# sThalham/PyraPose

Hardware: AMD Instinct MI355X
Metric: images/sec 640x480 fwd+bwd (train step: fwd + losses + bwd + clipnorm-Adam) (higher is better)
Workload: dtype bf16x3+f16c8

## Files before the change

include/pyrapose_hip.h:

```cpp
#ifndef PYRAPOSE_HIP_H
#define PYRAPOSE_HIP_H

#include <stddef.h>
#include <stdint.h>

#ifdef __cplusplus
extern "C" {
#endif

#define PP_OK 0
#define PP_ERR_ARG (-1)
#define PP_ERR_SHAPE (-2)
#define PP_ERR_ALIGN (-3)
#define PP_ERR_NOCTX (-4)
#define PP_ERR_UNSUPPORTED (-5)
#define PP_ERR_COMM (-6)

#define PP_MAX_SEG 5

typedef struct pp_ctx pp_ctx;

int pp_ctx_create(pp_ctx** out, int device, void* hip_stream);
void pp_ctx_destroy(pp_ctx* ctx);
int pp_ctx_set_stream(pp_ctx* ctx, void* hip_stream);
int pp_ctx_set_workspace(pp_ctx* ctx, void* device_buffer, size_t bytes);
int pp_ctx_set_split_capture(pp_ctx* ctx, void* hi, void* lo);
int pp_row_block_list(pp_ctx* ctx, const float* x, int rows, int ld, int cols, unsigned char* flags, int* list);
int pp_row_block_list_planes(pp_ctx* ctx, const void* x_hi, const void* x_lo, int rows, int ld, int cols, unsigned char* flags, int* list);
int pp_row_block_list_planes_within(pp_ctx* ctx, const void* x_hi, const void* x_lo, int rows, int ld, int cols, const unsigned char* within,
                                    unsigned char* flags, int* list);
int pp_ctx_set_epilogue_planes(pp_ctx* ctx, const void* add_hi, const void* add_lo, const void* mask_hi);
int pp_ctx_set_row_block_skip(pp_ctx* ctx, const unsigned char* flags, const int* list);
int pp_ctx_set_row_block_lazy(pp_ctx* ctx, int lazy_out, int lazy_in);
const char* pp_last_error_string(pp_ctx* ctx);
const char* pp_version(void);
int pp_device_info(pp_ctx* ctx, int* n_cu, char* name_host, int name_len);

typedef struct {
  int n_img;
  int n_seg;
  int h[PP_MAX_SEG];
  int w[PP_MAX_SEG];
} pp_rowspace;

typedef struct {
  pp_rowspace in;
  pp_rowspace out;
  int cin, cout;
  int kh, kw, stride;
  int pad_t, pad_l;
  int ld_x, ld_y, ld_w;
} pp_conv_desc;

int pp_conv2d_nhwc_fwd(pp_ctx* ctx, const pp_conv_desc* d, const float* x, const float* w,
                       const float* bias, const float* residual, int ld_res, int relu, float* y);

int pp_conv2d_nhwc_bwd_data(pp_ctx* ctx, const pp_conv_desc* d, const float* dy, const float* w,
                            const float* addend, int ld_add, const float* relu_src, int ld_rs, float* dx);

int pp_conv2d_nhwc_bwd_weight(pp_ctx* ctx, const pp_conv_desc* d, const float* x, const float* dy,
                              float* dw, float* dbias);

int pp_conv_split_weights_bf16x3(pp_ctx* ctx, const pp_conv_desc* d, const float* w, void* fwd_hi, void* fwd_lo,
                                 void* dgrad_hi, void* dgrad_lo);
typedef struct pp_split_job {
  const float* w;
  void* fwd_hi; void* fwd_lo; void* dg_hi; void* dg_lo;
  int taps, cin, cout, ld_w;
  int tile_begin, reserved;
} pp_split_job;
int pp_conv_split_weights_bf16x3_batch(pp_ctx* ctx, int n_jobs, const pp_split_job* jobs_dev, int total_tiles);
int pp_positive_row_blocks(pp_ctx* ctx, const pp_rowspace* rs, int A, int stride, const float* y_true, unsigned char* flags);
int pp_row_block_dilate(pp_ctx* ctx, const pp_conv_desc* d, const unsigned char* in_flags, unsigned char* out_flags);
int pp_ctx_set_row_block_out(pp_ctx* ctx, const unsigned char* flags, int* list);
int pp_split_planes_bf16x3(pp_ctx* ctx, size_t n, const float* src, void* hi, void* lo);
int pp_ctx_set_planes_format(pp_ctx* ctx, int fmt);
int pp_convert_planes(pp_ctx* ctx, size_t n, const void* src_hi, const void* src_lo, int src_fmt, void* dst_hi, void* dst_lo, int dst_fmt,
                      const float* scale2_dev, int scale_index, const void* relu_src_hi);
int pp_grad_scale_from_counts(pp_ctx* ctx, const int* counts_dev, int n_counts, float* scale2_dev);
int pp_grad_scale_from_counts_adj(pp_ctx* ctx, const int* counts_dev, int n_counts, float* scale2_dev, int log2_adjust);
int pp_split_planes_scaled_bf16x3(pp_ctx* ctx, size_t n, const float* src, void* hi, void* lo, const float* scale_dev);
int pp_ctx_set_grad_scale(pp_ctx* ctx, const float* scale2_dev);

int pp_conv2d_nhwc_fwd_bf16x3(pp_ctx* ctx, const pp_conv_desc* d, const float* x, const void* x_hi, const void* x_lo,
                              const void* w_fwd_hi, const void* w_fwd_lo, const float* bias, const float* residual,
                              int ld_res, int relu, float* y, void* y_hi, void* y_lo);
int pp_conv2d_nhwc_bwd_data_bf16x3(pp_ctx* ctx, const pp_conv_desc* d, const float* dy, const void* dy_hi,
                                   const void* dy_lo, const void* w_dgrad_hi, const void* w_dgrad_lo,
                                   const float* addend, int ld_add, const float* relu_src, int ld_rs, float* dx,
                                   void* dx_hi, void* dx_lo);
int pp_conv2d_nhwc_bwd_weight_bf16x3(pp_ctx* ctx, const pp_conv_desc* d, const float* x, const float* dy,
                                     const void* x_hi, const void* x_lo, const void* dy_hi, const void* dy_lo,
                                     float* dw, float* dbias);

typedef struct pp_comm pp_comm;
int pp_comm_available(void);
int pp_comm_unique_id(pp_ctx* ctx, void* id128);
int pp_comm_init(pp_ctx* ctx, int world, int rank, const void* id128, pp_comm** out);
int pp_comm_destroy(pp_comm* comm);
int pp_allreduce_bucket(pp_ctx* ctx, pp_comm* comm, float* buf, size_t count);
int pp_allreduce_counts(pp_ctx* ctx, pp_comm* comm, int* counts, int n);

int pp_maxpool3x3s2_fwd(pp_ctx* ctx, int n_img, int h, int w, int c, const float* x, int oh, int ow, float* y);
int pp_upsample_nearest_add_fwd(pp_ctx* ctx, int n_img, int sh, int sw, int th, int tw, int c,
                                const float* src, const float* other, float* out);
int pp_upsample_nearest_add_bwd(pp_ctx* ctx, int n_img, int sh, int sw, int th, int tw, int c,
                                const float* dtarget, const float* base, float* dsrc);
int pp_add_n(pp_ctx* ctx, size_t n, const float* a, const float* b, const float* c, float* out);
int pp_relu_fwd(pp_ctx* ctx, size_t n, const float* x, float* y);
typedef struct pp_tview {
  const float* f32;
  const void* hi;
  const void* lo;
} pp_tview;
int pp_add_n_v(pp_ctx* ctx, size_t n, const pp_tview* a, const pp_tview* b, const pp_tview* c, const pp_tview* out);
int pp_relu_fwd_v(pp_ctx* ctx, size_t n, const pp_tview* x, const pp_tview* y);
int pp_upsample_nearest_add_fwd_v(pp_ctx* ctx, int n_img, int sh, int sw, int th, int tw, int c, const pp_tview* src,
                                  const pp_tview* other, const pp_tview* out);
int pp_upsample_nearest_add_bwd_v(pp_ctx* ctx, int n_img, int sh, int sw, int th, int tw, int c, const pp_tview* dtarget,
                                  const pp_tview* base, const pp_tview* dsrc);
int pp_merge_planes_bf16x3(pp_ctx* ctx, size_t n, const void* hi, const void* lo, float* dst);
int pp_planes_stats(pp_ctx* ctx, const void* hi, const void* lo, long long rows, int ld, int cols, const unsigned char* within,
                    unsigned long long* stats5_dev);
int pp_pack_rgb_to_4(pp_ctx* ctx, size_t n_pixels, const float* x3, float* x4);
int pp_preprocess_caffe_u8(pp_ctx* ctx, int n_img, int H, int W, const int* sizes_hw_host, const unsigned char* images_u8,
                           float* x4);
int pp_warp_affine_u8(pp_ctx* ctx, int n_img, int H, int W, int channels, const double* mats_host, int interpolation, int border,
                      int cval, const unsigned char* src, unsigned char* dst);
int pp_resize_scale(int rows, int cols, int min_side, int max_side, double* scale);
int pp_resize_linear_u8(pp_ctx* ctx, int n_img, int SH, int SW, int channels, double scale, int DH, int DW, const unsigned char* src,
                        unsigned char* dst);
int pp_pack_rgb_to_4_padded(pp_ctx* ctx, int n_img, int H, int W, int Hp, int Wp, int pad, const float* x3, float* x4p);
int pp_preprocess_caffe_u8_padded(pp_ctx* ctx, int n_img, int H, int W, int Hp, int Wp, int pad, const int* sizes_hw_host,
                                  const unsigned char* images_u8, float* x4p);
int pp_stem7x7s2_fwd_bf16x3(pp_ctx* ctx, int n_img, int H, int W, int Hp, int Wp, const float* x4p, const void* w_hi,
                            const void* w_lo, int cout, const float* bias, int relu, float* y, int ld_y);

int pp_export_head(pp_ctx* ctx, const pp_rowspace* rs, int n_anchor, int n_val, const float* src, int ld,
                   int apply_sigmoid, float* out);

int pp_count_positives(pp_ctx* ctx, size_t rows_box, const float* y_box, size_t rows_cls, int c_cls,
                       const float* y_cls, size_t rows_mask, int c_mask, const float* y_mask, int* counts);
int pp_sigmoid_focal_fwd_bwd(pp_ctx* ctx, const pp_rowspace* rs, int n_anchor, int n_class,
                             const float* logits, int ld, const float* y_true, float alpha, float gamma,
                             const int* count, float loss_weight, float* loss_sum, float* dlogits);
int pp_orth_smoothl1_fwd_bwd(pp_ctx* ctx, const pp_rowspace* rs, int n_anchor, const float* pred, int ld,
                             const float* y_true, float weight, float sigma, const int* count,
                             float loss_weight, float* loss_sum, float* dpred);

typedef struct {
  long long offset;
  long long count;
  int ld;
  int trainable;
  long long scale_off;
  float l2;
} pp_param_desc;

typedef struct pp_optimizer pp_optimizer;
int pp_optimizer_create(pp_ctx* ctx, pp_optimizer** out, const pp_param_desc* descs_host, int n_desc,
                        long long total);
void pp_optimizer_destroy(pp_optimizer* opt);
int pp_grad_global_norm(pp_ctx* ctx, pp_optimizer* opt, const float* w_master, const float* g_eff,
                        const float* scales, float* gnorm_sq, float* l2_loss);
int pp_adam_step_clipnorm(pp_ctx* ctx, pp_optimizer* opt, float* w_master, float* w_eff, const float* g_eff,
                          const float* scales, float* m, float* v, const float* gnorm_sq, float lr,
                          float beta1, float beta2, float eps, float clipnorm, long long step);

int pp_generate_base_anchors_host(int base_size, const float* ratios_host, int n_ratios,
                                  const float* scales_host, int n_scales, double* out_host);
int pp_anchors_shift_f64(pp_ctx* ctx, int n_levels, const int* feat_h_host, const int* feat_w_host,
                         const int* strides_host, int n_anchor, const double* base_anchors_host,
                         double* anchors_out);
int pp_anchors_shift_f32(pp_ctx* ctx, int n_levels, const int* feat_h_host, const int* feat_w_host,
                         const int* strides_host, int n_anchor, const double* base_anchors_host,
                         float* anchors_out);
int pp_compute_overlap_f64(pp_ctx* ctx, int n, const double* boxes, int k, const double* query, double* overlaps);
int pp_compute_gt_annotations(pp_ctx* ctx, int n, const double* anchors, int k, const double* gt_boxes,
                              double negative_overlap, double positive_overlap, int* argmax, signed char* state);

int pp_anchor_targets(pp_ctx* ctx, int n_anchor_total, const double* anchors, int batch,
                      const int* gt_offset_host, const double* gt_boxes, const int* gt_labels,
                      const double* gt_box3d, const int* gt_mask_ids, const unsigned char* id_masks,
                      int mask_h, int mask_w, const int* mask_hw_host, const int* image_hw_host, int num_classes,
                      double negative_overlap, double positive_overlap, int out_mh, int out_mw,
                      float* regression, float* labels, float* mask);
// ... 65 lines not shown
```

pyrapose_amd/_lib.py:

```python
import ctypes as C
import os

_HERE = os.path.dirname(os.path.abspath(__file__))
LIB_PATH = os.path.join(_HERE, os.environ.get("PP_LIB") or "libpyrapose_hip.so")

PP_MAX_SEG = 5


class RowSpace(C.Structure):
    _fields_ = [("n_img", C.c_int), ("n_seg", C.c_int), ("h", C.c_int * PP_MAX_SEG), ("w", C.c_int * PP_MAX_SEG)]

    @classmethod
    def make(cls, n_img, shapes):
        rs = cls()
        rs.n_img = int(n_img)
        rs.n_seg = len(shapes)
        for i, (h, w) in enumerate(shapes):
            rs.h[i] = int(h)
            rs.w[i] = int(w)
        return rs

    def rows(self):
        return sum(self.n_img * self.h[i] * self.w[i] for i in range(self.n_seg))

    def shapes(self):
        return [(self.h[i], self.w[i]) for i in range(self.n_seg)]


class ConvDesc(C.Structure):
    _fields_ = [("in_", RowSpace), ("out", RowSpace), ("cin", C.c_int), ("cout", C.c_int), ("kh", C.c_int),
                ("kw", C.c_int), ("stride", C.c_int), ("pad_t", C.c_int), ("pad_l", C.c_int), ("ld_x", C.c_int),
                ("ld_y", C.c_int), ("ld_w", C.c_int)]


class ParamDesc(C.Structure):
    _fields_ = [("offset", C.c_longlong), ("count", C.c_longlong), ("ld", C.c_int), ("trainable", C.c_int),
                ("scale_off", C.c_longlong), ("l2", C.c_float)]


class SplitJob(C.Structure):
    _fields_ = [("w", C.c_void_p), ("fwd_hi", C.c_void_p), ("fwd_lo", C.c_void_p), ("dg_hi", C.c_void_p), ("dg_lo", C.c_void_p),
                ("taps", C.c_int), ("cin", C.c_int), ("cout", C.c_int), ("ld_w", C.c_int), ("tile_begin", C.c_int), ("reserved", C.c_int)]


class TView(C.Structure):
    _fields_ = [("f32", C.c_void_p), ("hi", C.c_void_p), ("lo", C.c_void_p)]


def _load():
    if not os.path.exists(LIB_PATH):
        raise ImportError(
            "pyrapose_amd: %s not found. Build it with `python -c 'import __graft_entry__ as g; g.build()'` "
            "or `make -C pyrapose_amd/csrc`. There is no CPU fallback." % LIB_PATH)
    try:
        return C.CDLL(LIB_PATH)
    except OSError as e:
        raise ImportError("pyrapose_amd: cannot load %s: %s" % (LIB_PATH, e))


lib = _load()

_p = C.c_void_p
_i = C.c_int
_f = C.c_float
_d = C.c_double
_ll = C.c_longlong
_sz = C.c_size_t

_SIGS = {
    "pp_ctx_create": (_i, [C.POINTER(_p), _i, _p]),
    "pp_ctx_destroy": (None, [_p]),
    "pp_ctx_set_stream": (_i, [_p, _p]),
    "pp_last_error_string": (C.c_char_p, [_p]),
    "pp_version": (C.c_char_p, []),
    "pp_device_info": (_i, [_p, C.POINTER(_i), C.c_char_p, _i]),
    "pp_conv2d_nhwc_fwd": (_i, [_p, C.POINTER(ConvDesc), _p, _p, _p, _p, _i, _i, _p]),
    "pp_conv2d_nhwc_bwd_data": (_i, [_p, C.POINTER(ConvDesc), _p, _p, _p, _i, _p, _i, _p]),
    "pp_conv2d_nhwc_bwd_weight": (_i, [_p, C.POINTER(ConvDesc), _p, _p, _p, _p]),
    "pp_conv_split_weights_bf16x3": (_i, [_p, C.POINTER(ConvDesc), _p, _p, _p, _p, _p]),
    "pp_split_planes_bf16x3": (_i, [_p, _sz, _p, _p, _p]),
    "pp_ctx_set_planes_format": (_i, [_p, _i]),
    "pp_convert_planes": (_i, [_p, _sz, _p, _p, _i, _p, _p, _i, _p, _i, _p]),
    "pp_split_planes_scaled_bf16x3": (_i, [_p, _sz, _p, _p, _p, _p]),
    "pp_grad_scale_from_counts": (_i, [_p, _p, _i, _p]),
    "pp_grad_scale_from_counts_adj": (_i, [_p, _p, _i, _p, _i]),
    "pp_ctx_set_grad_scale": (_i, [_p, _p]),
    "pp_planes_stats": (_i, [_p, _p, _p, _ll, _i, _i, _p, _p]),
    "pp_comm_available": (_i, []),
    "pp_comm_unique_id": (_i, [_p, _p]),
    "pp_comm_init": (_i, [_p, _i, _i, _p, C.POINTER(_p)]),
    "pp_comm_destroy": (_i, [_p]),
    "pp_allreduce_bucket": (_i, [_p, _p, _p, C.c_size_t]),
    "pp_allreduce_counts": (_i, [_p, _p, _p, _i]),
    "pp_ctx_set_workspace": (_i, [_p, _p, C.c_size_t]),
    "pp_ctx_set_split_capture": (_i, [_p, _p, _p]),
    "pp_row_block_list": (_i, [_p, _p, _i, _i, _i, _p, _p]),
    "pp_ctx_set_row_block_skip": (_i, [_p, _p, _p]),
    "pp_ctx_set_row_block_out": (_i, [_p, _p, _p]),
    "pp_ctx_set_row_block_lazy": (_i, [_p, _i, _i]),
    "pp_positive_row_blocks": (_i, [_p, _p, _i, _i, _p, _p]),
    "pp_row_block_dilate": (_i, [_p, _p, _p, _p]),
    "pp_row_block_list_planes": (_i, [_p, _p, _p, _i, _i, _i, _p, _p]),
    "pp_row_block_list_planes_within": (_i, [_p, _p, _p, _i, _i, _i, _p, _p, _p]),
    "pp_ctx_set_epilogue_planes": (_i, [_p, _p, _p, _p]),
    "pp_add_n_v": (_i, [_p, _sz, C.POINTER(TView), C.POINTER(TView), C.POINTER(TView), C.POINTER(TView)]),
    "pp_relu_fwd_v": (_i, [_p, _sz, C.POINTER(TView), C.POINTER(TView)]),
    "pp_upsample_nearest_add_fwd_v": (_i, [_p, _i, _i, _i, _i, _i, _i, C.POINTER(TView), C.POINTER(TView), C.POINTER(TView)]),
    "pp_upsample_nearest_add_bwd_v": (_i, [_p, _i, _i, _i, _i, _i, _i, C.POINTER(TView), C.POINTER(TView), C.POINTER(TView)]),
    "pp_merge_planes_bf16x3": (_i, [_p, _sz, _p, _p, _p]),
    "pp_warp_affine_u8": (_i, [_p, _i, _i, _i, _i, C.POINTER(_d), _i, _i, _i, _p, _p]),
    "pp_resize_scale": (_i, [_i, _i, _i, _i, C.POINTER(_d)]),
    "pp_resize_linear_u8": (_i, [_p, _i, _i, _i, _i, _d, _i, _i, _p, _p]),
    "pp_conv_split_weights_bf16x3_batch": (_i, [_p, _i, _p, _i]),
    "pp_conv2d_nhwc_fwd_bf16x3": (_i, [_p, C.POINTER(ConvDesc), _p, _p, _p, _p, _p, _p, _p, _i, _i, _p, _p, _p]),
    "pp_conv2d_nhwc_bwd_data_bf16x3": (_i, [_p, C.POINTER(ConvDesc), _p, _p, _p, _p, _p, _p, _i, _p, _i, _p, _p, _p]),
    "pp_conv2d_nhwc_bwd_weight_bf16x3": (_i, [_p, C.POINTER(ConvDesc), _p, _p, _p, _p, _p, _p, _p, _p]),
    "pp_maxpool3x3s2_fwd": (_i, [_p, _i, _i, _i, _i, _p, _i, _i, _p]),
    "pp_upsample_nearest_add_fwd": (_i, [_p, _i, _i, _i, _i, _i, _i, _p, _p, _p]),
    "pp_upsample_nearest_add_bwd": (_i, [_p, _i, _i, _i, _i, _i, _i, _p, _p, _p]),
    "pp_add_n": (_i, [_p, _sz, _p, _p, _p, _p]),
    "pp_relu_fwd": (_i, [_p, C.c_size_t, _p, _p]),
    "pp_preprocess_caffe_u8": (_i, [_p, _i, _i, _i, C.POINTER(C.c_int), _p, _p]),
    "pp_preprocess_caffe_u8_padded": (_i, [_p, _i, _i, _i, _i, _i, _i, C.POINTER(C.c_int), _p, _p]),
    "pp_pack_rgb_to_4_padded": (_i, [_p, _i, _i, _i, _i, _i, _i, _p, _p]),
    "pp_stem7x7s2_fwd_bf16x3": (_i, [_p, _i, _i, _i, _i, _i, _p, _p, _p, _i, _p, _i, _p, _i]),
    "pp_pack_rgb_to_4": (_i, [_p, _sz, _p, _p]),
    "pp_export_head": (_i, [_p, C.POINTER(RowSpace), _i, _i, _p, _i, _i, _p]),
    "pp_count_positives": (_i, [_p, _sz, _p, _sz, _i, _p, _sz, _i, _p, _p]),
    "pp_sigmoid_focal_fwd_bwd": (_i, [_p, C.POINTER(RowSpace), _i, _i, _p, _i, _p, _f, _f, _p, _f, _p, _p]),
    "pp_orth_smoothl1_fwd_bwd": (_i, [_p, C.POINTER(RowSpace), _i, _p, _i, _p, _f, _f, _p, _f, _p, _p]),
    "pp_optimizer_create": (_i, [_p, C.POINTER(_p), C.POINTER(ParamDesc), _i, _ll]),
    "pp_optimizer_destroy": (None, [_p]),
    "pp_grad_global_norm": (_i, [_p, _p, _p, _p, _p, _p, _p]),
    "pp_adam_step_clipnorm": (_i, [_p, _p, _p, _p, _p, _p, _p, _p, _p, _f, _f, _f, _f, _f, _ll]),
    "pp_generate_base_anchors_host": (_i, [_i, C.POINTER(_f), _i, C.POINTER(_f), _i, C.POINTER(_d)]),
    "pp_anchors_shift_f64": (_i, [_p, _i, C.POINTER(_i), C.POINTER(_i), C.POINTER(_i), _i, C.POINTER(_d), _p]),
    "pp_anchors_shift_f32": (_i, [_p, _i, C.POINTER(_i), C.POINTER(_i), C.POINTER(_i), _i, C.POINTER(_d), _p]),
    "pp_compute_overlap_f64": (_i, [_p, _i, _p, _i, _p, _p]),
    "pp_compute_gt_annotations": (_i, [_p, _i, _p, _i, _p, _d, _d, _p, _p]),
    "pp_anchor_targets": (_i, [_p, _i, _p, _i, C.POINTER(_i), _p, _p, _p, _p, _p, _i, _i, C.POINTER(_i), C.POINTER(_i), _i, _d, _d,
                               _i, _i, _p, _p, _p]),
    "pp_project_box3d_host": (_i, [C.POINTER(_d), C.POINTER(_d), C.POINTER(_d), C.POINTER(_d)]),
    "pp_pil_nearest_index_host": (_i, [_i, _i, C.POINTER(_i)]),
    "pp_box3d_decode": (_i, [_p, _i, _i, _p, _p, _p]),
    "pp_score_threshold_compact": (_i, [_p, _i, _i, _i, _p, _f, _i, _p, _p]),
    "pp_filter_workspace_bytes": (_sz, [_i, _i, _i]),
    "pp_pose_error_workspace_bytes": (_sz, [_i, _i]),
    "pp_filter_detections": (_i, [_p, _i, _i, _p, _p, _p, _f, _f, _i, _p, _p, _p, _p, _p]),
    "pp_pose_add_f64": (_i, [_p, _i, _i, _p, _p, _p, _p, _p, _p, _p]),
    "pp_pose_adi_f64": (_i, [_p, _i, _i, _p, _p, _p, _p, _p, _p, _p]),
    "pp_filter_detections_batch": (_i, [_p, _i, _i, _i, _p, _p, _p, _f, _f, _i, _p, _p, _p, _p, _p]),
    "pp_render_workspace_bytes": (_sz, [_i, _i, _i, _i, _i]),
    "pp_render_depth_f32": (_i, [_p, _i, _i, _p, _i, _p, _p, _p, _p, _i, _i, _d, _d, _p, _sz, _p]),
    "pp_vsd_workspace_bytes": (_sz, [_i, _i, _i]),
    "pp_vsd_f64": (_i, [_p, _i, _i, _i, _p, _ll, _p, _p, _p, _d, _d, _i, _p, _p, _p, _p]),
    "pp_pose_reproj_f64": (_i, [_p, _i, _i, _p, _p, _p, _p, _p, _p, _p, _p]),
    "pp_pnp_ransac_workspace_bytes": (_sz, [_i, _i]),
    "pp_pnp_ransac_f64": (_i, [_p, _i, _p, _i, _p, _p, _p, _i, _d, C.c_ulonglong, _i, _p, _p, _p, _p, _p, _p]),
    "pp_cloud_from_depth_workspace_bytes": (_sz, [_i, _i]),
    "pp_cloud_from_depth_f64": (_i, [_p, _i, _i, _p, _p, _i, _i, _p, _p, _d, _d, _d, _d, _d, _i, _p, _p, _p]),
    "pp_voxel_workspace_bytes": (_sz, [_i]),
    "pp_voxel_keys_f64": (_i, [_p, _i, _p, _d, _p, _p]),
    "pp_voxel_means_f64": (_i, [_p, _i, _p, _p, _p, _i, _p, _p, _p]),
    "pp_estimate_normals_workspace_bytes": (_sz, [_i, _i]),
    "pp_estimate_normals_f64": (_i, [_p, _i, _p, _d, _i, _p, _p, _p]),
    "pp_icp_workspace_bytes": (_sz, [_i, _i]),
    "pp_icp_f64": (_i, [_p, _i, _p, _p, _i, _p, _p, _p, _p, _d, _i, _d, _d, _i, _p, _sz, _p, _p, _p, _p, _p, _p, _p]),
}

EXPORTS = sorted(_SIGS)

MISSING = []
for _name, (_res, _args) in _SIGS.items():
    try:
        _fn = getattr(lib, _name)
    except AttributeError:
        if not os.environ.get("PP_LIB"):
            raise
        MISSING.append(_name)
        continue
    _fn.restype = _res
    _fn.argtypes = _args


def check(rc, ctx=None, what=""):
    if rc == 0:
        return
    msg = ""
    if ctx is not None:
        s = lib.pp_last_error_string(ctx)
        msg = s.decode("utf-8", "replace") if s else ""
    if rc < 0:
        raise ValueError("%s failed (%d): %s" % (what or "pyrapose_hip", rc, msg))
    raise RuntimeError("%s failed (hipError %d): %s" % (what or "pyrapose_hip", rc, msg))
```

pyrapose_amd/csrc/conv3.hip:

```cpp
#include "conv_common.h"
#include "conv4.h"

#define PP_CAT_(a, b) a##b
#define PP_CAT(a, b) PP_CAT_(a, b)
#if PP_FMT == 1
#define PP_API(name) PP_CAT(name, _fmt1)
#else
#define PP_API(name) PP_CAT(name, _fmt0)
#endif
namespace {
#include "planes_fmt.h"

#include "conv3_shared.h"

#ifndef PP_EPI_GF
#define PP_EPI_GF 4
#endif

template <int TM, int TN, bool AP, bool OP>
__global__ __launch_bounds__(256, (TM * TN >= 8) ? 2 : ((TM * TN == 4) ? 3 : 4)) void igemm3_kernel(
    const IgemmParams p, const float* __restrict__ g_src, const uint4* __restrict__ g_ahi, const uint4* __restrict__ g_alo,
    const uint4* __restrict__ g_whi, const uint4* __restrict__ g_wlo,
    const float* __restrict__ g_bias, const float* __restrict__ g_addend, const float* __restrict__ g_mask,
    float* __restrict__ g_out, uint2* __restrict__ g_ohi, uint2* __restrict__ g_olo, int w_rows, int w_ld8) {
// ... 664 lines not shown
    const int dx = p.off_x + TX * p.tsign;
    const unsigned tap_bits = (1u << (c_ty * 3 + TX)) * 0x10001u;
    const unsigned okm = f_valid & tap_bits;
    unsigned a_ok = 0;
#pragma unroll
    for (int a = 0; a < TM; ++a) a_ok |= (((okm >> (16 * (a & 1))) & 0xffffu) != 0 ? 1u : 0u) << a;
    if (VAR & 2) __builtin_amdgcn_s_setprio(1);
    mma_step<TM, TN, BM, BN, (VAR & 4) ? 2 : ((VAR & 1) ? 0 : 1), 1>(acc, Ahi, Ahi, Bhi, Bhi + NO * BN, wm * 32 * TM + il + dx, wn * 32 * TN + il, h, a_ok, 8 * BM);
    if (VAR & 2) __builtin_amdgcn_s_setprio(0);
  };
  std::integral_constant<int, 0> c0;
  std::integral_constant<int, 1> c1;
  auto tap_end = [&](auto n) {
    constexpr int N = decltype(n)::value;
    if constexpr (N == 0) asm volatile("s_waitcnt vmcnt(0)" ::: "memory");
    else if constexpr (N == 2) asm volatile("s_waitcnt vmcnt(2)" ::: "memory");
    else if constexpr (N == 4) asm volatile("s_waitcnt vmcnt(4)" ::: "memory");
    else if constexpr (N == 6) asm volatile("s_waitcnt vmcnt(6)" ::: "memory");
    else static_assert(N == 0, "tap_end: count");
    __builtin_amdgcn_s_barrier();
    asm volatile("" ::: "memory");
  };
  auto group = [&](int g, auto k) {
    constexpr int K = decltype(k)::value;
    const int c_ty = g % 3;
    const int gn = g + 1 < G ? g + 1 : 0;
    uint4* const Ahi = stA(std::integral_constant<int, K & 1>{});
    if constexpr (BST == 3) {
      dma_a(gn, stA(std::integral_constant<int, (K + 1) & 1>{}));
      dma_b(g, 2, sB2);
      mma_tile(c_ty, 0, Ahi, sB0);
      tap_end(std::integral_constant<int, 6>{});
      dma_b(gn, 0, sB0);
      mma_tile(c_ty, 1, Ahi, sB1);
      tap_end(std::integral_constant<int, 2>{});
      dma_b(gn, 1, sB1);
      mma_tile(c_ty, 2, Ahi, sB2);
      tap_end(std::integral_constant<int, 2>{});
    } else {
      constexpr int U = 3 * K;
      dma_b(g, 1, stB(std::integral_constant<int, (U + 1) & 1>{}));
      dma_a(gn, stA(std::integral_constant<int, (K + 1) & 1>{}));
      mma_tile(c_ty, 0, Ahi, stB(std::integral_constant<int, U & 1>{}));
      tap_end(std::integral_constant<int, 4>{});
      dma_b(g, 2, stB(std::integral_constant<int, U & 1>{}));
      mma_tile(c_ty, 1, Ahi, stB(std::integral_constant<int, (U + 1) & 1>{}));
      tap_end(std::integral_constant<int, 0>{});
      dma_b(gn, 0, stB(std::integral_constant<int, (U + 1) & 1>{}));
      mma_tile(c_ty, 2, Ahi, stB(std::integral_constant<int, U & 1>{}));
      tap_end(std::integral_constant<int, 0>{});
    }
  };

  if (tid == 0) {
    sA0[8 * BM] = make_uint4(0u, 0u, 0u, 0u);
    sA0[8 * BM + 1] = make_uint4(0u, 0u, 0u, 0u);
    sA1[8 * BM] = make_uint4(0u, 0u, 0u, 0u);
    sA1[8 * BM + 1] = make_uint4(0u, 0u, 0u, 0u);
  }
  if ((VAR & 8) && NWM == 4 && wave >= 4) __builtin_amdgcn_s_setprio(1);
  dma_a(0, sA0);
  dma_b(0, 0, sB0);
  if constexpr (BST == 3) {
    dma_b(0, 1, sB1);
    tap_end(std::integral_constant<int, 2>{});
  } else {
    tap_end(std::integral_constant<int, 0>{});
  }
  for (int g = 0; g < G; g += 2) {
    group(g, c0);
    if (g + 1 >= G) break;
    group(g + 1, c1);
  }
  asm volatile("s_waitcnt vmcnt(0)" ::: "memory");
  __syncthreads();
  epilogue3<TM, TN, OP, 4, false, true, false, NWM, 128 * NWM, (NWM == 2 ? 1 : 0)>(p, acc, sA0, m0, n0, tid, wm, wn, il, h, g_bias, g_addend, g_mask, g_out, g_ohi, g_olo);
}

__device__ __forceinline__ void finish4(const IgemmParams& p, float4 v, long long mo, int co, bool with_addend, const float* __restrict__ g_addend,
                                        const float* __restrict__ g_mask, float* __restrict__ g_out, void* __restrict__ g_ohi,
                                        void* __restrict__ g_olo) {
  if (with_addend) {
    if (p.add_hi) {
      const float4 a = planes_ld4(p.add_hi, p.add_lo, (mo * p.ld_add + co) >> 2);
      v.x += a.x; v.y += a.y; v.z += a.z; v.w += a.w;
    } else if (g_addend) {
      const float4 a = *reinterpret_cast<const float4*>(g_addend + mo * p.ld_add + co);
      v.x += a.x; v.y += a.y; v.z += a.z; v.w += a.w;
    }
  }
  if (p.mask_hi || g_mask) {
    const float4 k = p.mask_hi ? hi_ld4(p.mask_hi, (mo * p.ld_mask + co) >> 2) : *reinterpret_cast<const float4*>(g_mask + mo * p.ld_mask + co);
    v.x = k.x > 0.f ? v.x : 0.f; v.y = k.y > 0.f ? v.y : 0.f; v.z = k.z > 0.f ? v.z : 0.f; v.w = k.w > 0.f ? v.w : 0.f;
  }
  if (p.relu) { v.x = fmaxf(v.x, 0.f); v.y = fmaxf(v.y, 0.f); v.z = fmaxf(v.z, 0.f); v.w = fmaxf(v.w, 0.f); }
  if (g_out) *reinterpret_cast<float4*>(g_out + mo * p.ld_out + co) = v;
  if (g_ohi) planes_st4(g_ohi, g_olo, (mo * p.ld_out + co) >> 2, v);
}

__global__ void class_fill_kernel(const IgemmParams p, const float* __restrict__ g_addend, const float* __restrict__ g_mask,
                                  float* __restrict__ g_out, void* __restrict__ g_ohi, void* __restrict__ g_olo) {
  const int n4 = (p.Nout + 3) >> 2;
  const long long total = (long long)p.M * n4;
  const int hw = p.seg[0].OH * p.seg[0].OW;
  for (long long i = blockIdx.x * (long long)blockDim.x + threadIdx.x; i < total; i += (long long)gridDim.x * blockDim.x) {
    const int m = (int)(i / n4), co = 4 * (int)(i - (long long)m * n4);
    const int n = m / hw, rem = m - n * hw, yq = rem / p.seg[0].OW, xq = rem - yq * p.seg[0].OW;
    const long long mo = (long long)(n * p.sc_H + 2 * yq + p.sc_cy) * p.sc_W + 2 * xq + p.sc_cx;
    finish4(p, make_float4(0.f, 0.f, 0.f, 0.f), mo, co, true, g_addend, g_mask, g_out, g_ohi, g_olo);
  }
}

__global__ void splitk_finish_kernel(const IgemmParams p, int splits, const float* __restrict__ ws, const float* __restrict__ g_bias,
                                     const float* __restrict__ g_addend, const float* __restrict__ g_mask, float* __restrict__ g_out,
                                     void* __restrict__ g_ohi, void* __restrict__ g_olo) {
  const int n4 = (p.Nout + 3) >> 2;
  const int rows = p.M - p.m_off;
  const long long total = (long long)rows * n4, slice = (long long)rows * p.ld_out;
  for (long long i = blockIdx.x * (long long)blockDim.x + threadIdx.x; i < total; i += (long long)gridDim.x * blockDim.x) {
    const int mr = (int)(i / n4), co = 4 * (int)(i - (long long)mr * n4);
    const int m = p.m_off + mr;
    const float* w = ws + (long long)mr * p.ld_out + co;
    float4 v = *reinterpret_cast<const float4*>(w);
    for (int s = 1; s < splits; ++s) {
      const float4 q = *reinterpret_cast<const float4*>(w + s * slice);
      v.x += q.x; v.y += q.y; v.z += q.z; v.w += q.w;
    }
    if (g_bias) { const float4 b = *reinterpret_cast<const float4*>(g_bias + co); v.x += b.x; v.y += b.y; v.z += b.z; v.w += b.w; }
    finish4(p, v, (long long)m, co, true, g_addend, g_mask, g_out, g_ohi, g_olo);
  }
}

__global__ void rl_splitk_finish_kernel(const IgemmParams p, int splits, const float* __restrict__ ws, const int* __restrict__ g_rl,
                                        const float* __restrict__ g_bias, const float* __restrict__ g_addend, const float* __restrict__ g_mask,
                                        float* __restrict__ g_out, void* __restrict__ g_ohi, void* __restrict__ g_olo) {
  const int j = blockIdx.x;
  if (j >= g_rl[0]) return;
  const int n4 = (p.Nout + 3) >> 2;
  const long long slice = (((long long)p.M + 31) & ~31ll) * p.ld_out;
  const int m0 = g_rl[1 + j] * 32, nr = min(32, p.M - m0);
  for (int i = threadIdx.x; i < nr * n4; i += blockDim.x) {
    const int r = i / n4, co = 4 * (i - r * n4);
    const float* w = ws + ((long long)j * 32 + r) * p.ld_out + co;
    float4 v = *reinterpret_cast<const float4*>(w);
    for (int s = 1; s < splits; ++s) {
      const float4 q = *reinterpret_cast<const float4*>(w + s * slice);
      v.x += q.x; v.y += q.y; v.z += q.z; v.w += q.w;
    }
    if (g_bias) { const float4 b = *reinterpret_cast<const float4*>(g_bias + co); v.x += b.x; v.y += b.y; v.z += b.z; v.w += b.w; }
    finish4(p, v, (long long)(m0 + r), co, true, g_addend, g_mask, g_out, g_ohi, g_olo);
  }
}

__global__ void split_planes_kernel(size_t n8, const float4* __restrict__ src, uint4* __restrict__ hi, uint4* __restrict__ lo,
                                    const float* __restrict__ scale) {
  const float sc = scale ? *scale : 1.f;
  for (size_t i = blockIdx.x * (size_t)blockDim.x + threadIdx.x; i < n8; i += (size_t)gridDim.x * blockDim.x) {
    uint4 h, l;
    float4 a = src[2 * i], b = src[2 * i + 1];
    a.x *= sc; a.y *= sc; a.z *= sc; a.w *= sc;
    b.x *= sc; b.y *= sc; b.z *= sc; b.w *= sc;
    split8(a, b, &h, &l);
    hi[2 * i] = h;
    lo[2 * i] = l;
  }
}

__global__ void grad_scale_kernel(const int* __restrict__ counts, int n_counts, float* __restrict__ scale2, int base_log2) {
  if (threadIdx.x == 0 && blockIdx.x == 0) {
    int n = 0x7fffffff;
    for (int i = 0; i < n_counts; ++i) n = counts[i] < n ? counts[i] : n;
    n = n < 1 ? 1 : n;
    int e = 0;
    while ((n >> (e + 1)) != 0) ++e;
    const float s = __uint_as_float((unsigned)(127 + base_log2 + e) << 23);
    scale2[0] = s;
    scale2[1] = 1.f / s;
  }
}

__global__ void row_block_flags_kernel(const float* __restrict__ x, int rows, int ld, int cols4, unsigned char* __restrict__ flags) {
  const int blk = blockIdx.x, r0 = blk * 32;
  const int nr = rows - r0 < 32 ? rows - r0 : 32;
  int any = 0;
  for (int i = threadIdx.x; i < nr * cols4; i += blockDim.x) {
    const int r = i / cols4, c = i - r * cols4;
    const float4 v = *reinterpret_cast<const float4*>(x + (long long)(r0 + r) * ld + 4 * c);
    any |= (v.x != 0.f) | (v.y != 0.f) | (v.z != 0.f) | (v.w != 0.f);
  }
  any = __syncthreads_or(any);
  if (threadIdx.x == 0) flags[blk] = any ? 1 : 0;
}

__global__ void row_block_flags_planes_kernel(const uint2* __restrict__ hi, const uint2* __restrict__ lo, int rows, int ld4, int cols4,
                                              unsigned char* __restrict__ flags, const unsigned char* __restrict__ within) {
  const int blk = blockIdx.x, r0 = blk * 32;
  if (within && !within[blk]) {
    if (threadIdx.x == 0) flags[blk] = 0;
    return;
  }
  const int nr = rows - r0 < 32 ? rows - r0 : 32;
  int any = 0;
  for (int i = threadIdx.x; i < nr * cols4; i += blockDim.x) {
    const int r = i / cols4, c = i - r * cols4;
    const long long o = pk4((long long)(r0 + r) * ld4 + c);
    const uint2 h = hi[o], l = lo[o];
    any |= fmt_any_nonzero(h.x | h.y, l.x | l.y) ? 1 : 0;
  }
  any = __syncthreads_or(any);
  if (threadIdx.x == 0) flags[blk] = any ? 1 : 0;
}

__global__ void row_block_compact_kernel(const unsigned char* __restrict__ flags, int n_blocks, int* __restrict__ list) {
  __shared__ int wave_cnt[4];
  __shared__ int base;
  const int tid = threadIdx.x, lane = tid & 63, wave = tid >> 6;
  if (tid == 0) base = 0;
  __syncthreads();
  for (int i0 = 0; i0 < n_blocks; i0 += 256) {
    const int i = i0 + tid;
    const bool f = i < n_blocks && flags[i] != 0;
    const unsigned long long m = __ballot(f);
    const int before = __popcll(m & ((1ull << lane) - 1ull));
    if (lane == 0) wave_cnt[wave] = __popcll(m);
    __syncthreads();
    int off = base;
    for (int w = 0; w < wave; ++w) off += wave_cnt[w];
    if (f) list[1 + off + before] = i;
    __syncthreads();
    if (tid == 0) base += wave_cnt[0] + wave_cnt[1] + wave_cnt[2] + wave_cnt[3];
    __syncthreads();
  }
  if (tid == 0) list[0] = base;
}

}
extern "C" int PP_API(pp_row_block_list)(pp_ctx* ctx, const float* x, int rows, int ld, int cols, unsigned char* flags, int* list) {
  PP_REQUIRE_CTX(ctx);
  PP_CHECK_ARG(ctx, x && flags && list && rows > 0 && cols > 0 && cols <= ld && ld % 4 == 0 && pp_is_aligned16(x), PP_ERR_ARG,
               "pp_row_block_list: bad tensor (ld %% 4 == 0, 16-byte aligned)");
  const int nb = (rows + 31) / 32, cols4 = (cols + 3) / 4;
  PP_CHECK_ARG(ctx, 4 * cols4 <= ld, PP_ERR_SHAPE, "pp_row_block_list: cols rounded up to 4 exceed ld");
  hipLaunchKernelGGL(row_block_flags_kernel, dim3((unsigned)nb), dim3(256), 0, ctx->stream, x, rows, ld, cols4, flags);
  hipLaunchKernelGGL(row_block_compact_kernel, dim3(1), dim3(256), 0, ctx->stream, (const unsigned char*)flags, nb, list);
  PP_CHECK_LAUNCH(ctx, "pp_row_block_list");
  return PP_OK;
}
namespace {

}
extern "C" int PP_API(pp_row_block_list_planes_within)(pp_ctx* ctx, const void* x_hi, const void* x_lo, int rows, int ld, int cols,
                                               const unsigned char* within, unsigned char* flags, int* list);
namespace {
}
extern "C" int PP_API(pp_row_block_list_planes)(pp_ctx* ctx, const void* x_hi, const void* x_lo, int rows, int ld, int cols, unsigned char* flags,
                                        int* list) {
  return PP_API(pp_row_block_list_planes_within)(ctx, x_hi, x_lo, rows, ld, cols, nullptr, flags, list);
}
namespace {

}
extern "C" int PP_API(pp_row_block_list_planes_within)(pp_ctx* ctx, const void* x_hi, const void* x_lo, int rows, int ld, int cols,
                                               const unsigned char* within, unsigned char* flags, int* list) {
  PP_REQUIRE_CTX(ctx);
  PP_CHECK_ARG(ctx, x_hi && x_lo && flags && list && rows > 0 && cols > 0 && cols <= ld && ld % 8 == 0 && pp_is_packed(x_hi, x_lo), PP_ERR_ARG,
               "pp_row_block_list_planes: bad tensor (ld %% 8 == 0, packed planes)");
  const int nb = (rows + 31) / 32, cols4 = (cols + 3) / 4;
  PP_CHECK_ARG(ctx, 4 * cols4 <= ld, PP_ERR_SHAPE, "pp_row_block_list_planes: cols rounded up to 4 exceed ld");
  hipLaunchKernelGGL(row_block_flags_planes_kernel, dim3((unsigned)nb), dim3(256), 0, ctx->stream, (const uint2*)x_hi, (const uint2*)x_lo, rows,
                     ld / 4, cols4, flags, within);
  hipLaunchKernelGGL(row_block_compact_kernel, dim3(1), dim3(256), 0, ctx->stream, (const unsigned char*)flags, nb, list);
  PP_CHECK_LAUNCH(ctx, "pp_row_block_list_planes");
  return PP_OK;
}
namespace {

static int split_planes_impl(pp_ctx* ctx, size_t n, const float* src, void* hi, void* lo, const float* scale);
}
extern "C" int PP_API(pp_split_planes_bf16x3)(pp_ctx* ctx, size_t n, const float* src, void* hi, void* lo) {
  return split_planes_impl(ctx, n, src, hi, lo, nullptr);
}
namespace {
}
extern "C" int PP_API(pp_split_planes_scaled_bf16x3)(pp_ctx* ctx, size_t n, const float* src, void* hi, void* lo, const float* scale_dev) {
  return split_planes_impl(ctx, n, src, hi, lo, scale_dev);
}
namespace {
}
extern "C" int PP_API(pp_grad_scale_from_counts_adj)(pp_ctx* ctx, const int* counts_dev, int n_counts, float* scale2_dev, int log2_adjust) {
  PP_REQUIRE_CTX(ctx);
  PP_CHECK_ARG(ctx, counts_dev && scale2_dev && n_counts >= 1 && n_counts <= 16 && log2_adjust >= -16 && log2_adjust <= 16, PP_ERR_ARG,
               "pp_grad_scale_from_counts: bad arguments");
  static const int base_log2 = []() { const char* e = getenv("PP_GSCALE_LOG2"); const int v = e ? atoi(e) : 8; return v < -20 ? -20 : (v > 30 ? 30 : v); }();
  hipLaunchKernelGGL(grad_scale_kernel, dim3(1), dim3(64), 0, ctx->stream, counts_dev, n_counts, scale2_dev, base_log2 + log2_adjust);
  PP_CHECK_LAUNCH(ctx, "pp_grad_scale_from_counts");
  return PP_OK;
}
extern "C" int PP_API(pp_grad_scale_from_counts)(pp_ctx* ctx, const int* counts_dev, int n_counts, float* scale2_dev) {
  return PP_API(pp_grad_scale_from_counts_adj)(ctx, counts_dev, n_counts, scale2_dev, 0);
}
namespace {
static int split_planes_impl(pp_ctx* ctx, size_t n, const float* src, void* hi, void* lo, const float* scale) {
  PP_REQUIRE_CTX(ctx);
  PP_CHECK_ARG(ctx, src && hi && lo && n % 8 == 0, PP_ERR_ARG, "pp_split_planes_bf16x3: n must be a multiple of 8");
  PP_CHECK_ARG(ctx, pp_is_aligned16(src) && pp_is_packed(hi, lo), PP_ERR_ALIGN, "pp_split_planes_bf16x3: alignment / packed planes (lo = hi + 16 bytes)");
  if (n == 0) return PP_OK;
  size_t blocks = (n / 8 + 255) / 256;
  const size_t cap = (size_t)(ctx->n_cu > 0 ? ctx->n_cu : 256) * 8;
  if (blocks > cap) blocks = cap;
  hipLaunchKernelGGL(split_planes_kernel, dim3((unsigned)blocks), dim3(256), 0, ctx->stream, n / 8, (const float4*)src, (uint4*)hi, (uint4*)lo, scale);
  PP_CHECK_LAUNCH(ctx, "pp_split_planes_bf16x3");
  return PP_OK;
}

__device__ __forceinline__ void split_weights_tile(int tap, int ci0, int co0, int cin, int cout, int ld_w, const float* __restrict__ w,
                                                   unsigned short* __restrict__ fwd_hi, unsigned short* __restrict__ fwd_lo, int cout_rows,
                                                   unsigned short* __restrict__ dg_hi, unsigned short* __restrict__ dg_lo, int dg_ld) {
  __shared__ unsigned short t_hi[32][33], t_lo[32][33];
  const int tx = threadIdx.x, ty = threadIdx.y;
  for (int j = ty; j < 32; j += 8) {
    const int ci = ci0 + j, co = co0 + tx;
    float v = 0.f;
    if (ci < cin && co < cout) v = w[((long long)tap * cin + ci) * ld_w + co];
    unsigned short uh, ul;
    fmt_encode_weight(v, &uh, &ul);
    t_hi[j][tx] = uh;
    t_lo[j][tx] = ul;
    if (dg_hi && ci < cin && co < dg_ld) {
      const long long o = ((long long)tap * cin + ci) * dg_ld + co;
      dg_hi[o] = uh;
      dg_lo[o] = ul;
    }
  }
  __syncthreads();
  if (fwd_hi) {
    for (int j = ty; j < 32; j += 8) {
      const int co = co0 + j, ci = ci0 + tx;
      if (co < cout_rows && ci < cin) {
        const long long o = ((long long)tap * cout_rows + co) * cin + ci;
        fwd_hi[o] = t_hi[tx][j];
        fwd_lo[o] = t_lo[tx][j];
      }
    }
  }
}

__global__ void split_weights_kernel(int taps, int cin, int cout, int ld_w, const float* __restrict__ w,
                                     unsigned short* __restrict__ fwd_hi, unsigned short* __restrict__ fwd_lo, int cout_rows,
                                     unsigned short* __restrict__ dg_hi, unsigned short* __restrict__ dg_lo, int dg_ld) {
  split_weights_tile(blockIdx.z, blockIdx.y * 32, blockIdx.x * 32, cin, cout, ld_w, w, fwd_hi, fwd_lo, cout_rows, dg_hi, dg_lo, dg_ld);
}

__global__ void split_weights_batch_kernel(int n_jobs, const pp_split_job* __restrict__ jobs) {
  int lo = 0, hi = n_jobs - 1;
  while (lo < hi) {
    const int mid = (lo + hi + 1) >> 1;
    if (jobs[mid].tile_begin <= (int)blockIdx.x) lo = mid; else hi = mid - 1;
  }
  const pp_split_job j = jobs[lo];
  const int dg_ld = (j.cout + 31) / 32 * 32;
  const int tiles_co = dg_ld / 32, tiles_ci = j.cin / 32;
  int t = (int)blockIdx.x - j.tile_begin;
  const int co_t = t % tiles_co;
  t /= tiles_co;
  const int ci_t = t % tiles_ci, tap = t / tiles_ci;
  split_weights_tile(tap, ci_t * 32, co_t * 32, j.cin, j.cout, j.ld_w, j.w, (unsigned short*)j.fwd_hi, (unsigned short*)j.fwd_lo, j.cout,
                     (unsigned short*)j.dg_hi, (unsigned short*)j.dg_lo, dg_ld);
}

}
extern "C" int PP_API(pp_conv_split_weights_bf16x3_batch)(pp_ctx* ctx, int n_jobs, const pp_split_job* jobs_dev, int total_tiles) {
  PP_REQUIRE_CTX(ctx);
  PP_CHECK_ARG(ctx, n_jobs >= 0 && total_tiles >= 0 && (n_jobs == 0 || jobs_dev), PP_ERR_ARG, "pp_conv_split_weights_bf16x3_batch: bad arguments");
  if (n_jobs == 0 || total_tiles == 0) return PP_OK;
  hipLaunchKernelGGL(split_weights_batch_kernel, dim3((unsigned)total_tiles), dim3(32, 8), 0, ctx->stream, n_jobs, jobs_dev);
  PP_CHECK_LAUNCH(ctx, "pp_conv_split_weights_bf16x3_batch");
  return PP_OK;
}
namespace {

}
extern "C" int PP_API(pp_conv_split_weights_bf16x3)(pp_ctx* ctx, const pp_conv_desc* d, const float* w, void* fwd_hi, void* fwd_lo,
                                            void* dg_hi, void* dg_lo) {
  PP_REQUIRE_CTX(ctx);
  int rc = check_desc(ctx, d, "pp_conv_split_weights_bf16x3");
  if (rc) return rc;
  PP_CHECK_ARG(ctx, w && ((fwd_hi && fwd_lo) || (dg_hi && dg_lo)), PP_ERR_ARG, "pp_conv_split_weights_bf16x3: null tensor");
  PP_CHECK_ARG(ctx, d->cin % 32 == 0, PP_ERR_SHAPE, "pp_conv_split_weights_bf16x3: cin %d must be a multiple of 32", d->cin);
  const int taps = d->kh * d->kw;
  const int dg_ld = (d->cout + 31) / 32 * 32;
  dim3 grid((unsigned)((dg_ld + 31) / 32), (unsigned)((d->cin + 31) / 32), (unsigned)taps);
  hipLaunchKernelGGL(split_weights_kernel, grid, dim3(32, 8), 0, ctx->stream, taps, d->cin, d->cout, d->ld_w, w,
                     (unsigned short*)fwd_hi, (unsigned short*)fwd_lo, d->cout, (unsigned short*)dg_hi, (unsigned short*)dg_lo, dg_ld);
  PP_CHECK_LAUNCH(ctx, "pp_conv_split_weights_bf16x3");
  return PP_OK;
}
namespace {

static bool igemm3_fast_ok(const IgemmParams& p, bool planes, int w_rows, int w_ld8) {
  static const bool fast_on = []() { const char* e = getenv("PP_CONV3_FAST"); return !(e && e[0] == '0'); }();
  const long long a_bytes = p.src_rows * (long long)p.ld_src * 4;
  (void)planes;
  const long long w_bytes = (long long)p.w_taps * w_rows * w_ld8 * 16;
  int max_sw = 0;
  for (int i = 0; i < p.n_seg; ++i) max_sw = p.seg[i].SW > max_sw ? p.seg[i].SW : max_sw;
  return fast_on && p.div == 1 && p.kh * p.kw <= 31 && a_bytes < (1ll << 31) && w_bytes < (1ll << 31) &&
         (long long)max_sw * p.ld_src * 4 < (1ll << 23) && p.src_rows > 0;
}

static bool igemm3x_ok(const IgemmParams& p, bool planes_in, bool planes_out, int w_rows, int w_ld8) {
  static const bool x_on = []() { const char* e = getenv("PP_CONV3_XREUSE"); return !(e && e[0] == '0'); }();
  bool same = x_on && igemm3_fast_ok(p, planes_in, w_rows, w_ld8) && !p.sc_on && p.kw == 3 && p.mul == 1 && p.div == 1 &&
              (p.src != nullptr || planes_in) && (!planes_in || p.ld_src % 8 == 0) && p.w_tstep == 1 && p.w_tx0 == 0;
  (void)planes_out;
  for (int i = 0; i < p.n_seg && same; ++i)
    same = p.seg[i].OH == p.seg[i].SH && p.seg[i].OW == p.seg[i].SW && p.seg[i].row_begin == p.seg[i].src_row_begin;
  return same;
}

__global__ void rl_dilate_kernel(const IgemmParams p, const unsigned char* __restrict__ in_flags, unsigned char* __restrict__ out_flags,
                                 int n_blocks) {
  const int b = blockIdx.x * blockDim.x + threadIdx.x;
  if (b >= n_blocks) return;
  const int r_lo = 32 * b, r_hi = min(32 * b + 31, p.M - 1);
  int any = 0;
  for (int s = 0; s < p.n_seg; ++s) {
    const int seg_lo = p.seg[s].row_begin, seg_hi = (s + 1 < p.n_seg ? p.seg[s + 1].row_begin : p.M) - 1;
    if (r_hi < seg_lo || r_lo > seg_hi) continue;
    const int W = p.seg[s].OW;
    for (int j = -1; j <= 1; ++j) {
      int lo = r_lo - 1 + j * W, hi = r_hi + 1 + j * W;
      lo = lo < 0 ? 0 : lo;
      hi = hi > p.M - 1 ? p.M - 1 : hi;
      for (int q = lo >> 5; q <= (hi >> 5); ++q) any |= in_flags[q];
    }
  }
  out_flags[b] = any ? 1 : 0;
}

__global__ void rl_fill_kernel(const IgemmParams p, const unsigned char* __restrict__ live, const float* __restrict__ g_addend,
                               const float* __restrict__ g_mask, float* __restrict__ g_out, void* __restrict__ g_ohi, void* __restrict__ g_olo) {
  const int b = blockIdx.x;
  if (live[b]) return;
  const int n4 = (p.Nout + 3) >> 2;
  const int r0 = 32 * b, nr = min(32, p.M - r0);
  if (g_ohi && !g_out && !g_addend && p.Nout == p.ld_out && (p.ld_out & 7) == 0 && (p.add_hi == nullptr || (p.ld_add & 7) == 0) &&
      (p.mask_hi == nullptr || (p.ld_mask & 7) == 0)) {
    const int n8 = nr * (p.ld_out >> 3);
    uint4* dst = reinterpret_cast<uint4*>(g_ohi) + 2 * (long long)r0 * (p.ld_out >> 3);
    const uint4 z4 = make_uint4(0u, 0u, 0u, 0u);
    for (int i = threadIdx.x; i < n8; i += blockDim.x) {
      uint4 oh = z4, ol = z4;
      if (p.add_hi) {
        const int r = i / (p.ld_out >> 3), g8 = i - r * (p.ld_out >> 3);
        const uint4* a = reinterpret_cast<const uint4*>(p.add_hi) + 2 * ((long long)(r0 + r) * (p.ld_add >> 3) + g8);
        oh = a[0];
        ol = a[1];
        if (p.mask_hi) {
          const uint4 k = reinterpret_cast<const uint4*>(p.mask_hi)[2 * ((long long)(r0 + r) * (p.ld_mask >> 3) + g8)];
          const unsigned kk[4] = {k.x, k.y, k.z, k.w};
          unsigned hh[4] = {oh.x, oh.y, oh.z, oh.w}, ll[4] = {ol.x, ol.y, ol.z, ol.w};
#pragma unroll
          for (int j = 0; j < 4; ++j) {
            const unsigned lo_ok = ((kk[j] & 0x8000u) == 0u && (kk[j] & 0x7fffu) != 0u) ? 0x0000ffffu : 0u;
            const unsigned hi_ok = ((kk[j] & 0x80000000u) == 0u && (kk[j] & 0x7fff0000u) != 0u) ? 0xffff0000u : 0u;
            hh[j] &= (lo_ok | hi_ok);
            ll[j] &= (lo_ok | hi_ok);
          }
          oh = make_uint4(hh[0], hh[1], hh[2], hh[3]);
          ol = make_uint4(ll[0], ll[1], ll[2], ll[3]);
        }
      }
      dst[2 * i] = oh;
      dst[2 * i + 1] = ol;
    }
    return;
  }
  for (int i = threadIdx.x; i < nr * n4; i += blockDim.x) {
    const int r = i / n4, co = 4 * (i - r * n4);
    const long long m = r0 + r;
    const float4 z = make_float4(0.f, 0.f, 0.f, 0.f);
    if (g_addend || p.add_hi) {
      finish4(p, z, m, co, true, g_addend, g_mask, g_out, g_ohi, g_olo);
    } else {
      if (g_out) *reinterpret_cast<float4*>(g_out + m * p.ld_out + co) = z;
      if (g_ohi) {
        reinterpret_cast<uint2*>(g_ohi)[pk4((m * p.ld_out + co) >> 2)] = make_uint2(0u, 0u);
        reinterpret_cast<uint2*>(g_olo)[pk4((m * p.ld_out + co) >> 2)] = make_uint2(0u, 0u);
      }
    }
  }
}

__global__ void row_block_compact_kernel(const unsigned char* __restrict__ flags, int n_blocks, int* __restrict__ list);

template <int TM, int TN>
static void launch_igemm3_rowlist(hipStream_t st, IgemmParams& p, const void* ahi, const void* alo, const void* whi, const void* wlo, int w_rows,
                                  int w_ld8, void* ohi, void* olo, const unsigned char* dy_flags, unsigned char* out_flags, int* out_list,
                                  float* ws, size_t ws_bytes, bool fill = true) {
  constexpr int BM = 64 * TM, BN = 64 * TN;
  const int nb = (p.M + 31) / 32;
  static const int want_splits = []() { const char* e = getenv("PP_SPARSE_DGRAD_SPLITS"); return e ? atoi(e) : 2; }();
  const int n_steps = p.kh * p.kw * (p.Cred / 32);
  int splits = 1;
  if (ws && want_splits > 1 && (ohi || p.out)) {
    const long long slice_bytes = (long long)nb * 32 * p.ld_out * 4;
    splits = want_splits;
    while (splits > 1 && (n_steps / splits < 24 || slice_bytes * splits > (long long)ws_bytes)) --splits;
  }
  if (dy_flags) hipLaunchKernelGGL(rl_dilate_kernel, dim3((unsigned)((nb + 255) / 256)), dim3(256), 0, st, p, dy_flags, out_flags, nb);
  hipLaunchKernelGGL(row_block_compact_kernel, dim3(1), dim3(256), 0, st, (const unsigned char*)out_flags, nb, out_list);
  p.n_tiles_n = (p.Nout + BN - 1) / BN;
  const int n_tiles_m = (nb + BM / 32 - 1) / (BM / 32);
  const long long a_bytes = p.src_rows * (long long)p.ld_src * 4, w_bytes = (long long)p.w_taps * w_rows * w_ld8 * 16;
  const dim3 grid((unsigned)(n_tiles_m * p.n_tiles_n * splits));
  if (ahi && !ohi)
    hipLaunchKernelGGL((igemm3f_kernel<TM, TN, true, false, false, true>), grid, dim3(256), 0, st, p, ahi, alo, (unsigned)a_bytes, whi, wlo,
                       (unsigned)w_bytes, p.bias, p.addend, p.mask_src, p.out, (uint2*)nullptr, (uint2*)nullptr, w_rows, w_ld8, splits,
                       splits > 1 ? ws : (float*)nullptr, (const int*)out_list, dy_flags);
  else if (ahi)
    hipLaunchKernelGGL((igemm3f_kernel<TM, TN, true, true, false, true>), grid, dim3(256), 0, st, p, ahi, alo, (unsigned)a_bytes, whi, wlo,
                       (unsigned)w_bytes, p.bias, p.addend, p.mask_src, p.out, (uint2*)ohi, (uint2*)olo, w_rows, w_ld8, splits,
                       splits > 1 ? ws : (float*)nullptr, (const int*)out_list, dy_flags);
  else
    hipLaunchKernelGGL((igemm3f_kernel<TM, TN, false, false, false, true>), grid, dim3(256), 0, st, p, (const void*)p.src, nullptr,
                       (unsigned)a_bytes, whi, wlo, (unsigned)w_bytes, p.bias, p.addend, p.mask_src, p.out, (uint2*)nullptr, (uint2*)nullptr,
                       w_rows, w_ld8, splits, splits > 1 ? ws : (float*)nullptr, (const int*)out_list, dy_flags);
  if (splits > 1)
    hipLaunchKernelGGL(rl_splitk_finish_kernel, dim3((unsigned)nb), dim3(256), 0, st, p, splits, (const float*)ws, (const int*)out_list, p.bias,
                       p.addend, p.mask_src, p.out, ohi, olo);
  const bool in_place = (ohi != nullptr && p.add_hi == (const void*)ohi && p.ld_add == p.ld_out && !p.out && !p.addend && !p.mask_hi &&
                         !p.mask_src && !p.relu) ||
                        (p.out != nullptr && p.addend == p.out && p.ld_add == p.ld_out && !ohi && !p.add_hi && !p.mask_hi && !p.mask_src && !p.relu);
  if (fill && !in_place)
    hipLaunchKernelGGL(rl_fill_kernel, dim3((unsigned)nb), dim3(256), 0, st, p, (const unsigned char*)out_flags, p.addend, p.mask_src, p.out, ohi,
                       olo);
}

static void split_capture_pass(hipStream_t st, const IgemmParams& p, void* chi, void* clo) {
  const size_t n8 = (size_t)(p.src_rows * (long long)p.ld_src / 8);
  size_t blocks = (n8 + 255) / 256;
  if (blocks > 8192) blocks = 8192;
  hipLaunchKernelGGL(split_planes_kernel, dim3((unsigned)blocks), dim3(256), 0, st, n8, (const float4*)p.src, (uint4*)chi, (uint4*)clo, (const float*)nullptr);
}

template <int TM, int TN>
static void launch_igemm3(hipStream_t st, IgemmParams& p, const void* ahi, const void* alo, const void* whi, const void* wlo, int w_rows,
                          int w_ld8, void* ohi, void* olo, int splits, float* ws, void* chi = nullptr, void* clo = nullptr,
                          const unsigned char* flags = nullptr, float* ws_any = nullptr, size_t ws_any_bytes = 0, int n_cu = 256) {
  constexpr int BM = 64 * TM, BN = 64 * TN;
  p.n_tiles_n = (p.Nout + BN - 1) / BN;
  const int n_tiles_m = (p.M + BM - 1) / BM;
  const dim3 grid((unsigned)(n_tiles_m * p.n_tiles_n * splits));
  const bool fast = igemm3_fast_ok(p, ahi != nullptr, w_rows, w_ld8);
  const long long a_bytes = p.src_rows * (long long)p.ld_src * 4;
  const long long w_bytes = (long long)p.w_taps * w_rows * w_ld8 * 16;
  if (p.sc_on) {
    if (ahi)
      hipLaunchKernelGGL((igemm3f_kernel<TM, TN, true, true, true>), grid, dim3(256), 0, st, p, ahi, alo, (unsigned)a_bytes, whi, wlo,
                         (unsigned)w_bytes, p.bias, p.addend, p.mask_src, p.out, (uint2*)ohi, (uint2*)olo, w_rows, w_ld8, 1, nullptr);
    else
      hipLaunchKernelGGL((igemm3f_kernel<TM, TN, false, false, true>), grid, dim3(256), 0, st, p, (const void*)p.src, nullptr, (unsigned)a_bytes,
                         whi, wlo, (unsigned)w_bytes, p.bias, p.addend, p.mask_src, p.out, (uint2*)nullptr, (uint2*)nullptr, w_rows, w_ld8, 1,
                         nullptr);
    return;
  }
  {
    if (igemm3x_ok(p, ahi != nullptr, ohi != nullptr, w_rows, w_ld8) && (TM <= 2 || (ahi != nullptr && !chi))) {
      const int n_tiles_mx = (p.M + BM - 3) / (BM - 2);
      int skip_halo = 0;
      for (int i = 0; i < p.n_seg; ++i) skip_halo = p.seg[i].SW + 1 > skip_halo ? p.seg[i].SW + 1 : skip_halo;
      const dim3 gridx((unsigned)(n_tiles_mx * p.n_tiles_n * splits));
      static const int x_order = []() { const char* e = getenv("PP_CONV3_X_ORDER"); return e ? atoi(e) : 1; }();
      p.x_ty_inner = x_order;
      const bool op = ohi != nullptr && splits == 1;
      if constexpr (TM <= 2) {
        if (chi) {
          hipLaunchKernelGGL((igemm3x_kernel<TM, TN, true>), gridx, dim3(256), 0, st, p, (const void*)p.src, nullptr, (unsigned)a_bytes, whi, wlo,
                             (unsigned)w_bytes, p.bias, p.addend, p.mask_src, p.out, (uint2*)nullptr, (uint2*)nullptr, w_rows, w_ld8, splits,
                             ws, chi, clo, flags, skip_halo);
          return;
        }
      }
      if constexpr (TM == 2 && TN == 2) {
        const char* const dma_env = getenv("PP_CONV3_DMA");
        const bool dma_on = !(dma_env && dma_env[0] == '0');
        if (dma_on && ahi && op && !flags && splits == 1 && p.kh == 3 && x_order == 1 && w_rows % 128 == 0 && p.Cred % 32 == 0) {
          constexpr int BM4 = 256;
          const int n_tiles_m4 = (p.M + BM4 - 3) / (BM4 - 2);
          const int ntn = (p.Nout + 127) / 128;
          static const int dma_min = []() { const char* e = getenv("PP_CONV3_DMA_MIN"); return e ? atoi(e) : 512; }();
          static const int dma_frac = []() { const char* e = getenv("PP_CONV3_DMA_FRAC"); return e ? atoi(e) : 1000; }();
          const int n_blk = n_tiles_m4 * ntn;
          const bool one_and_a_bit = n_blk > n_cu && n_blk < 2 * n_cu && (n_blk - n_cu) * 100 >= dma_frac * n_cu;
          if (n_blk >= dma_min || one_and_a_bit) {
            static const bool tail_on = []() { const char* e = getenv("PP_CONV3_DMA_TAIL"); return !(e && e[0] == '0'); }();
            int full_rt = n_tiles_m4;
            const int rounds = (n_tiles_m4 * ntn) / n_cu;
            static const int tail_frac = []() { const char* e = getenv("PP_CONV3_DMA_TAIL_FRAC"); return e ? atoi(e) : 60; }();
            const int last = (n_tiles_m4 * ntn) % n_cu;
            if (tail_on && last != 0 && last * 100 < tail_frac * n_cu && rounds >= 2 && ws_any != nullptr) full_rt = rounds * n_cu / ntn;
            const int m_split = full_rt * (BM4 - 2);
            int tail_splits = 0;
            if (full_rt < n_tiles_m4) {
              const int rem = p.M - m_split;
              const int n_rt = (rem + BM - 3) / (BM - 2);
              const int groups = p.kh * (p.Cred / 32);
              int sp = (3 * n_cu + n_rt * ntn - 1) / (n_rt * ntn);
              while (sp > 1 && (groups / sp < 4 || (size_t)sp * rem * p.ld_out * 4 > ws_any_bytes)) --sp;
              if (sp > 1) tail_splits = sp;
              else full_rt = n_tiles_m4;
            }
            p.n_tiles_n = ntn;
            const char* const e_var = getenv("PP_CONV3_DMA_VAR");
            const int var = e_var ? atoi(e_var) : 1;
            auto go4 = [&](auto v) {
              hipLaunchKernelGGL((igemm4x_kernel<true, decltype(v)::value>), dim3((unsigned)(full_rt * ntn)), dim3(512), 0, st, p, ahi, alo,
                                 (unsigned)a_bytes, whi, wlo, (unsigned)w_bytes, p.bias, p.addend, p.mask_src, p.out, (uint2*)ohi, (uint2*)olo, w_rows,
                                 w_ld8);
            };
            if (var == 0) go4(std::integral_constant<int, 0>{});
            else if (var == 2) go4(std::integral_constant<int, 2>{});
            else if (var == 3) go4(std::integral_constant<int, 3>{});
            else if (var == 4) go4(std::integral_constant<int, 4>{});
            else if (var == 9) go4(std::integral_constant<int, 9>{});
            else go4(std::integral_constant<int, 1>{});
            if (tail_splits > 1) {
              IgemmParams q = p;
              q.m_off = full_rt * (BM4 - 2);
              const int rem = q.M - q.m_off;
              const int n_rt = (rem + BM - 3) / (BM - 2);
              hipLaunchKernelGGL((igemm3x_kernel<TM, TN, false, true, false>), dim3((unsigned)(n_rt * ntn * tail_splits)), dim3(256), 0, st, q, ahi,
                                 alo, (unsigned)a_bytes, whi, wlo, (unsigned)w_bytes, q.bias, q.addend, q.mask_src, q.out, (uint2*)nullptr,
                                 (uint2*)nullptr, w_rows, w_ld8, tail_splits, ws_any, nullptr, nullptr, (const unsigned char*)nullptr, skip_halo);
              const long long total = (long long)rem * ((q.Nout + 3) >> 2);
              long long blocks = (total + 255) / 256;
              if (blocks > (long long)n_cu * 8) blocks = (long long)n_cu * 8;
              hipLaunchKernelGGL(splitk_finish_kernel, dim3((unsigned)blocks), dim3(256), 0, st, q, tail_splits, (const float*)ws_any, q.bias, q.addend,
                                 q.mask_src, q.out, ohi, olo);
            }
            return;
          }
          const char* const e_dma2 = getenv("PP_CONV3_DMA2");
          const bool dma2_on = e_dma2 && e_dma2[0] == '1';
          static const int dma2_min = []() { const char* e = getenv("PP_CONV3_DMA2_MIN"); return e ? atoi(e) : 512; }();
          if (dma2_on && n_tiles_mx * ntn >= dma2_min) {
            p.n_tiles_n = ntn;
            hipLaunchKernelGGL((igemm4x_kernel<true, 1, 2>), dim3((unsigned)(n_tiles_mx * ntn)), dim3(256), 0, st, p, ahi, alo, (unsigned)a_bytes, whi,
                               wlo, (unsigned)w_bytes, p.bias, p.addend, p.mask_src, p.out, (uint2*)ohi, (uint2*)olo, w_rows, w_ld8);
            return;
          }
        }
      }
      if (ahi && op)
        hipLaunchKernelGGL((igemm3x_kernel<TM, TN, false, true, true>), gridx, dim3(256), 0, st, p, ahi, alo, (unsigned)a_bytes, whi, wlo,
                           (unsigned)w_bytes, p.bias, p.addend, p.mask_src, p.out, (uint2*)ohi, (uint2*)olo, w_rows, w_ld8, splits, ws, nullptr,
                           nullptr, flags, skip_halo);
      else if (ahi)
        hipLaunchKernelGGL((igemm3x_kernel<TM, TN, false, true, false>), gridx, dim3(256), 0, st, p, ahi, alo, (unsigned)a_bytes, whi, wlo,
                           (unsigned)w_bytes, p.bias, p.addend, p.mask_src, p.out, (uint2*)nullptr, (uint2*)nullptr, w_rows, w_ld8, splits, ws,
                           nullptr, nullptr, flags, skip_halo);
      else if constexpr (TM <= 2) {
        if (op)
          hipLaunchKernelGGL((igemm3x_kernel<TM, TN, false, false, true>), gridx, dim3(256), 0, st, p, (const void*)p.src, nullptr,
                             (unsigned)a_bytes, whi, wlo, (unsigned)w_bytes, p.bias, p.addend, p.mask_src, p.out, (uint2*)ohi, (uint2*)olo,
                             w_rows, w_ld8, splits, ws, nullptr, nullptr, flags, skip_halo);
        else
          hipLaunchKernelGGL((igemm3x_kernel<TM, TN, false>), gridx, dim3(256), 0, st, p, (const void*)p.src, nullptr, (unsigned)a_bytes, whi,
                             wlo, (unsigned)w_bytes, p.bias, p.addend, p.mask_src, p.out, (uint2*)nullptr, (uint2*)nullptr, w_rows, w_ld8, splits,
                             ws, nullptr, nullptr, flags, skip_halo);
      }
      return;
    }
  }
  if (chi) split_capture_pass(st, p, chi, clo);
  if (splits > 1) ohi = olo = nullptr;
  auto go = [&](auto ap, auto op) {
    constexpr bool AP = decltype(ap)::value, OP = decltype(op)::value;
    if (fast)
      hipLaunchKernelGGL((igemm3f_kernel<TM, TN, AP, OP>), grid, dim3(256), 0, st, p, AP ? ahi : (const void*)p.src, AP ? alo : nullptr,
                         (unsigned)a_bytes, whi, wlo, (unsigned)w_bytes, p.bias, p.addend, p.mask_src, p.out, (uint2*)ohi, (uint2*)olo,
                         w_rows, w_ld8, splits, ws);
    else
      hipLaunchKernelGGL((igemm3_kernel<TM, TN, AP, OP>), grid, dim3(256), 0, st, p, p.src, (const uint4*)(AP ? ahi : nullptr),
                         (const uint4*)(AP ? alo : nullptr), (const uint4*)whi, (const uint4*)wlo, p.bias, p.addend, p.mask_src, p.out,
                         (uint2*)ohi, (uint2*)olo, w_rows, w_ld8);
// ... 9 lines not shown
  static const double eff[5] = {1.1, 1.0, 0.9, 0.9, 0.8};
  static const int slots[5] = {2, 3, 4, 4, 4};
  static const int split_cand[8] = {1, 2, 3, 4, 6, 8, 12, 16};
  const int cus = ctx->n_cu > 0 ? ctx->n_cu : 256;
  const long long ws_bytes = (long long)ctx->ws_bytes;
  double best = 1e300;
  *splits = 1;
  for (int i = 0; i < 5; ++i) {
    const int bm = 64 * cand[i][0], bn = 64 * cand[i][1];
    const long long blocks = (long long)((M + bm - 1) / bm) * ((Nout + bn - 1) / bn);
    for (int si = 0; si < (may_split ? 8 : 1); ++si) {
      const int sp = split_cand[si];
      if (sp > 1 && (n_steps / sp < 8 || (long long)sp * M * ld_out * 4 > ws_bytes)) break;
      const double steps = (double)((n_steps + sp - 1) / sp) + 8.0;
      double t = est_rounds(blocks * sp, slots[i], cus) * steps * cand[i][0] * cand[i][1] / eff[i];
      if (sp > 1) {
        const double us = (double)M * Nout * (8.0 * sp + 12.0) / 4.0e6 + 4.0;
        t += us / 2.1 * 4.0;
      }
      if (t < best * 0.97) {
        best = t;
        *tm = cand[i][0];
        *tn = cand[i][1];
        *splits = sp;
      }
    }
  }
  static const bool x4 = []() { const char* e = getenv("PP_CONV3_X4"); return e && e[0] == '1'; }();
  if (x_ok && *tm == 4 && *splits == 1 && !x4) {
    *tm = 2;
    *tn = 2;
  }
  const char* e = getenv("PP_CONV3_TILE");
  if (e && e[0] && e[1] == ',' && e[2]) {
    *tm = e[0] - '0';
    *tn = e[2] - '0';
  }
  if (const char* es = getenv("PP_CONV3_SPLITS")) {
    const int v = atoi(es);
    if (v >= 1 && (v == 1 || (may_split && n_steps / v >= 1 && (long long)v * M * ld_out * 4 <= ws_bytes))) *splits = v;
  }
}

static void dispatch3(pp_ctx* ctx, IgemmParams& p, const void* ahi, const void* alo, const void* whi, const void* wlo, int w_rows,
                      int w_ld8, void* ohi, void* olo, void* chi = nullptr, void* clo = nullptr, const unsigned char* flags = nullptr) {
  int tm, tn, splits;
  const int n_steps = p.kh * p.kw * (p.Cred / 32);
  {
    const char* const e_on = getenv("PP_CONV4P");
    const char* const e_nst = getenv("PP_CONV4P_NST");
    const char* const e_sp = getenv("PP_CONV4P_SPLITS");
    const bool p_on = e_on && e_on[0] == '1';
    const int p_nst = e_nst && atoi(e_nst) == 3 ? 3 : 4;
    const int p_splits = e_sp ? atoi(e_sp) : 0;
    const long long a_bytes = p.src_rows * (long long)p.ld_src * 4, w_bytes = (long long)p.w_taps * w_rows * w_ld8 * 16;
    if (p_on && p.kh == 1 && p.kw == 1 && ahi && !chi && !flags && !p.sc_on && p.div == 1 && p.Cred % 32 == 0 && p.ld_src % 8 == 0 &&
        a_bytes < (1ll << 31) && w_bytes < (1ll << 31) && p.src_rows > 0 && (ohi || p.out)) {
      const int n_cu = ctx->n_cu > 0 ? ctx->n_cu : 256;
      const long long tiles = (long long)((p.M + 127) / 128) * ((p.Nout + 127) / 128);
      int sp = 1;
      if (tiles * 4 < (long long)n_cu * 3 && ctx->ws != nullptr) {
        sp = (int)(n_cu / tiles);
        while (sp > 1 && (n_steps / sp < 4 || (long long)sp * p.M * p.ld_out * 4 > (long long)ctx->ws_bytes)) --sp;
      }
      if (p_splits >= 1 && (p_splits == 1 || (ctx->ws != nullptr && n_steps / p_splits >= 1 && (long long)p_splits * p.M * p.ld_out * 4 <= (long long)ctx->ws_bytes)))
        sp = p_splits;
      if (getenv("PP_CONV_DEBUG"))
        fprintf(stderr, "igemm4p M %d N %d steps %d -> %lld tiles x %d splits on %d CUs, %d stages\n", p.M, p.Nout, n_steps, tiles, sp, n_cu, p_nst);
      PP_API(pp4_launch_igemm4p)(ctx->stream, p, ahi, whi, wlo, w_rows, w_ld8, ohi, olo, sp, sp > 1 ? ctx->ws : nullptr, n_cu, p_nst);
      if (sp > 1) {
        const long long total = (long long)p.M * ((p.Nout + 3) >> 2);
        long long blocks = (total + 255) / 256;
        if (blocks > (long long)n_cu * 8) blocks = (long long)n_cu * 8;
        hipLaunchKernelGGL(splitk_finish_kernel, dim3((unsigned)blocks), dim3(256), 0, ctx->stream, p, sp, ctx->ws, p.bias, p.addend, p.mask_src, p.out,
                           ohi, olo);
      }
      return;
    }
  }
  const bool may_split = ctx->ws != nullptr && (ohi || p.out != nullptr) && !p.sc_on && igemm3_fast_ok(p, ahi != nullptr, w_rows, w_ld8);
  pick_tile3(ctx, p.M, p.Nout, p.ld_out, n_steps, may_split, igemm3x_ok(p, ahi != nullptr, ohi != nullptr, w_rows, w_ld8), &tm, &tn, &splits);
  if (getenv("PP_CONV_DEBUG"))
    fprintf(stderr, "igemm3 M %d N %d steps %d -> tile %dx%d splits %d (may_split %d: ws %d planes_out %d out %d)\n", p.M, p.Nout, n_steps, 64 * tm,
            64 * tn, splits, (int)may_split, (int)(ctx->ws != nullptr), (int)(ohi != nullptr), (int)(p.out != nullptr));
  float* ws = splits > 1 ? ctx->ws : nullptr;
  if (tm == 4) launch_igemm3<4, 2>(ctx->stream, p, ahi, alo, whi, wlo, w_rows, w_ld8, ohi, olo, splits, ws, chi, clo, flags);
  else if (tm == 2 && tn == 2)
    launch_igemm3<2, 2>(ctx->stream, p, ahi, alo, whi, wlo, w_rows, w_ld8, ohi, olo, splits, ws, chi, clo, flags, ctx->ws, (size_t)ctx->ws_bytes,
                        ctx->n_cu > 0 ? ctx->n_cu : 256);
  else if (tm == 1 && tn == 2) launch_igemm3<1, 2>(ctx->stream, p, ahi, alo, whi, wlo, w_rows, w_ld8, ohi, olo, splits, ws, chi, clo, flags);
  else if (tm == 2 && tn == 1) launch_igemm3<2, 1>(ctx->stream, p, ahi, alo, whi, wlo, w_rows, w_ld8, ohi, olo, splits, ws, chi, clo, flags);
  else launch_igemm3<1, 1>(ctx->stream, p, ahi, alo, whi, wlo, w_rows, w_ld8, ohi, olo, splits, ws, chi, clo, flags);
  if (splits > 1) {
    const long long total = (long long)p.M * ((p.Nout + 3) >> 2);
    long long blocks = (total + 255) / 256;
    const long long cap = (long long)(ctx->n_cu > 0 ? ctx->n_cu : 256) * 8;
    if (blocks > cap) blocks = cap;
    hipLaunchKernelGGL(splitk_finish_kernel, dim3((unsigned)blocks), dim3(256), 0, ctx->stream, p, splits, ctx->ws, p.bias, p.addend, p.mask_src,
                       p.out, ohi, olo);
  }
}

}
extern "C" int PP_API(pp_conv2d_nhwc_fwd_bf16x3)(pp_ctx* ctx, const pp_conv_desc* d, const float* x, const void* x_hi, const void* x_lo,
                                         const void* w_hi, const void* w_lo, const float* bias, const float* residual, int ld_res,
                                         int relu, float* y, void* y_hi, void* y_lo) {
  PP_REQUIRE_CTX(ctx);
  void *chi = ctx->cap_hi, *clo = ctx->cap_lo;
  ctx->cap_hi = ctx->cap_lo = nullptr;
  const void *ep_ah = ctx->ep_add_hi, *ep_al = ctx->ep_add_lo;
  ctx->ep_add_hi = ctx->ep_add_lo = ctx->ep_mask_hi = nullptr;
  const unsigned char* out_flags = ctx->out_flags;
  int* out_list = ctx->out_list;
  ctx->out_flags = nullptr;
  ctx->out_list = nullptr;
  int rc = check_desc(ctx, d, "pp_conv2d_nhwc_fwd_bf16x3");
  PP_CHECK_ARG(ctx, !(ep_ah && residual), PP_ERR_ARG, "pp_conv2d_nhwc_fwd_bf16x3: residual given both as f32 and as planes");
  PP_CHECK_ARG(ctx, !ep_ah || (ld_res % 4 == 0 && ld_res >= ((d->cout + 3) & ~3)), PP_ERR_SHAPE, "pp_conv2d_nhwc_fwd_bf16x3: residual planes");
  if (rc) return rc;
  PP_CHECK_ARG(ctx, !chi || (x && !x_hi && pp_is_packed(chi, clo)), PP_ERR_ARG, "pp_conv2d_nhwc_fwd_bf16x3: split capture needs the f32 operand");
  PP_CHECK_ARG(ctx, (x || (x_hi && x_lo)) && w_hi && w_lo && (y || (y_hi && y_lo)), PP_ERR_ARG, "pp_conv2d_nhwc_fwd_bf16x3: null tensor");
  PP_CHECK_ARG(ctx, (x_hi == nullptr) == (x_lo == nullptr), PP_ERR_ARG, "pp_conv2d_nhwc_fwd_bf16x3: x_hi and x_lo go together");
  PP_CHECK_ARG(ctx, d->cin % 32 == 0 && d->ld_x % 8 == 0, PP_ERR_SHAPE, "pp_conv2d_nhwc_fwd_bf16x3: cin %d must be a multiple of 32, ld_x of 8", d->cin);
  PP_CHECK_ARG(ctx, pp_is_packed(x_hi, x_lo) && pp_is_packed(y_hi, y_lo) && pp_is_packed(ep_ah, ep_al), PP_ERR_ALIGN,
               "pp_conv2d_nhwc_fwd_bf16x3: planes must be packed (lo = hi + 16 bytes, 16-byte aligned)");
  PP_CHECK_ARG(ctx, !y_hi || (d->cout % 8 == 0 && d->ld_y % 8 == 0), PP_ERR_SHAPE, "pp_conv2d_nhwc_fwd_bf16x3: output planes need cout, ld_y %% 8 == 0");
  PP_CHECK_ARG(ctx, !ep_ah || (ld_res % 8 == 0 && d->cout % 8 == 0), PP_ERR_SHAPE, "pp_conv2d_nhwc_fwd_bf16x3: residual planes need cout, ld_res %% 8 == 0");
  PP_CHECK_ARG(ctx, (!x || pp_is_aligned16(x)) && pp_is_aligned16(w_hi) && pp_is_aligned16(w_lo) && (!y || pp_is_aligned16(y)), PP_ERR_ALIGN,
               "pp_conv2d_nhwc_fwd_bf16x3: tensors must be 16-byte aligned");
  PP_CHECK_ARG(ctx, !residual || (ld_res % 4 == 0 && ld_res >= ((d->cout + 3) & ~3) && pp_is_aligned16(residual)), PP_ERR_SHAPE,
               "pp_conv2d_nhwc_fwd_bf16x3: residual");
  PP_CHECK_ARG(ctx, !bias || pp_is_aligned16(bias), PP_ERR_ALIGN, "pp_conv2d_nhwc_fwd_bf16x3: bias alignment");
  IgemmParams p;
  memset(&p, 0, sizeof(p));
  p.src = x; p.out = y; p.bias = bias; p.addend = residual; p.mask_src = nullptr;
  p.add_hi = ep_ah; p.add_lo = ep_al;
  p.ld_src = d->ld_x; p.ld_w = d->ld_w; p.ld_out = d->ld_y; p.ld_add = ld_res; p.ld_mask = 0;
  p.relu = relu;
  p.n_seg = d->in.n_seg;
  fill_segs(ctx, d, true, p.seg, &p.M, &p.src_rows);
  p.Cred = d->cin; p.Nout = d->cout; p.w_tap_rows = d->cin;
  p.kh = d->kh; p.kw = d->kw;
  p.mul = d->stride; p.tsign = 1; p.off_y = -d->pad_t; p.off_x = -d->pad_l; p.div = 1;
  p.w_ty0 = 0; p.w_tx0 = 0; p.w_tstep = 1; p.w_kw = d->kw; p.w_taps = d->kh * d->kw;
  PP_CHECK_ARG(ctx, (y_hi == nullptr) == (y_lo == nullptr) && (!y_hi || (d->ld_y % 4 == 0 && pp_is_aligned16(y_hi) && pp_is_aligned16(y_lo))),
               PP_ERR_ARG, "pp_conv2d_nhwc_fwd_bf16x3: output planes");
  if (out_flags) {
    bool ok = x_hi != nullptr && ((y != nullptr) != (y_hi != nullptr)) && !chi && !residual && !ep_ah && d->stride == 1 && d->kh == 3 && d->kw == 3 && d->pad_t == 1 &&
              d->pad_l == 1 && igemm3_fast_ok(p, true, d->cout, d->cin / 8);
    for (int i = 0; i < p.n_seg && ok; ++i)
      ok = p.seg[i].OH == p.seg[i].SH && p.seg[i].OW == p.seg[i].SW && p.seg[i].row_begin == p.seg[i].src_row_begin;
    PP_CHECK_ARG(ctx, ok, PP_ERR_SHAPE, "pp_conv2d_nhwc_fwd_bf16x3: the row-block-out hint needs a 3x3 stride-1 'same' conv on plane-stored input");
    launch_igemm3_rowlist<2, 2>(ctx->stream, p, x_hi, x_lo, w_hi, w_lo, d->cout, d->cin / 8, y_hi, y_lo, nullptr, const_cast<unsigned char*>(out_flags),
                                out_list, ctx->ws, ctx->ws_bytes, false);
    PP_CHECK_LAUNCH(ctx, "pp_conv2d_nhwc_fwd_bf16x3");
    return PP_OK;
  }
  dispatch3(ctx, p, x_hi, x_lo, w_hi, w_lo, d->cout, d->cin / 8, y_hi, y_lo, chi, clo);
  PP_CHECK_LAUNCH(ctx, "pp_conv2d_nhwc_fwd_bf16x3");
  return PP_OK;
}
namespace {

}
extern "C" int PP_API(pp_row_block_dilate)(pp_ctx* ctx, const pp_conv_desc* d, const unsigned char* in_flags, unsigned char* out_flags) {
  PP_REQUIRE_CTX(ctx);
  int rc = check_desc(ctx, d, "pp_row_block_dilate");
  if (rc) return rc;
  PP_CHECK_ARG(ctx, in_flags && out_flags && in_flags != out_flags, PP_ERR_ARG, "pp_row_block_dilate: two distinct flag buffers");
  IgemmParams p;
  memset(&p, 0, sizeof(p));
  p.n_seg = d->in.n_seg;
  fill_segs(ctx, d, true, p.seg, &p.M, &p.src_rows);
  bool same = d->stride == 1 && d->kh == 3 && d->kw == 3;
  for (int i = 0; i < p.n_seg && same; ++i) same = p.seg[i].OH == p.seg[i].SH && p.seg[i].OW == p.seg[i].SW && p.seg[i].row_begin == p.seg[i].src_row_begin;
  PP_CHECK_ARG(ctx, same, PP_ERR_SHAPE, "pp_row_block_dilate: 3x3 stride-1 conv on an unchanged grid");
  const int nb = (p.M + 31) / 32;
  hipLaunchKernelGGL(rl_dilate_kernel, dim3((unsigned)((nb + 255) / 256)), dim3(256), 0, ctx->stream, p, in_flags, out_flags, nb);
  PP_CHECK_LAUNCH(ctx, "pp_row_block_dilate");
  return PP_OK;
}
namespace {

}
extern "C" int PP_API(pp_stem7x7s2_fwd_bf16x3)(pp_ctx* ctx, int n_img, int H, int W, int Hp, int Wp, const float* x4p, const void* w_hi,
                                       const void* w_lo, int cout, const float* bias, int relu, float* y, int ld_y) {
  PP_REQUIRE_CTX(ctx);
  PP_CHECK_ARG(ctx, x4p && w_hi && w_lo && y && pp_is_aligned16(x4p) && pp_is_aligned16(y) && pp_is_aligned16(w_hi) && pp_is_aligned16(w_lo),
               PP_ERR_ARG, "pp_stem7x7s2_fwd_bf16x3: null / unaligned tensor");
  PP_CHECK_ARG(ctx, n_img > 0 && H > 0 && W > 0 && Hp >= H + 6 && Wp >= W + 8 && Wp % 2 == 0 && cout > 0 && ld_y % 4 == 0 && ld_y >= ((cout + 3) & ~3),
               PP_ERR_SHAPE, "pp_stem7x7s2_fwd_bf16x3: bad geometry");
  const int OH = (H + 6 - 7) / 2 + 1, OW = (W + 6 - 7) / 2 + 1;
  IgemmParams p;
  memset(&p, 0, sizeof(p));
  p.src = x4p; p.out = y; p.bias = bias;
  p.ld_src = 4; p.ld_out = ld_y;
  p.relu = relu;
  p.n_seg = 1;
  p.seg[0].row_begin = 0; p.seg[0].src_row_begin = 0;
  p.seg[0].OH = OH; p.seg[0].OW = OW; p.seg[0].SH = Hp; p.seg[0].SW = Wp;
  p.M = n_img * OH * OW;
  p.src_rows = (long long)n_img * Hp * Wp;
  p.Cred = 32; p.Nout = cout; p.w_tap_rows = 32;
  p.kh = 7; p.kw = 1;
  p.mul = 2; p.tsign = 1; p.off_y = 0; p.off_x = 0; p.div = 1;
  p.w_ty0 = 0; p.w_tx0 = 0; p.w_tstep = 1; p.w_kw = 1; p.w_taps = 7;
  PP_CHECK_ARG(ctx, igemm3_fast_ok(p, false, cout, 4), PP_ERR_SHAPE, "pp_stem7x7s2_fwd_bf16x3: frame too large for 31-bit offsets");
  dispatch3(ctx, p, nullptr, nullptr, w_hi, w_lo, cout, 4, nullptr, nullptr);
  PP_CHECK_LAUNCH(ctx, "pp_stem7x7s2_fwd_bf16x3");
  return PP_OK;
}
namespace {

}
extern "C" int PP_API(pp_conv2d_nhwc_bwd_data_bf16x3)(pp_ctx* ctx, const pp_conv_desc* d, const float* dy, const void* dy_hi, const void* dy_lo,
                                              const void* w_hi, const void* w_lo, const float* addend, int ld_add,
                                              const float* relu_src, int ld_rs, float* dx, void* dx_hi, void* dx_lo) {
  PP_REQUIRE_CTX(ctx);
  void *chi = ctx->cap_hi, *clo = ctx->cap_lo;
  ctx->cap_hi = ctx->cap_lo = nullptr;
  const unsigned char* skip_flags = ctx->skip_flags;
  const int* skip_list_in = ctx->skip_list;
  const bool skip_scratch_ok = skip_flags != nullptr && skip_list_in != nullptr;
  ctx->skip_flags = nullptr;
  ctx->skip_list = nullptr;
  const bool lazy_out = ctx->lazy_out != 0, lazy_in = ctx->lazy_in != 0;
  ctx->lazy_out = ctx->lazy_in = 0;
  const void *ep_ah = ctx->ep_add_hi, *ep_al = ctx->ep_add_lo, *ep_mh = ctx->ep_mask_hi;
  ctx->ep_add_hi = ctx->ep_add_lo = ctx->ep_mask_hi = nullptr;
  int rc = check_desc(ctx, d, "pp_conv2d_nhwc_bwd_data_bf16x3");
  PP_CHECK_ARG(ctx, !(ep_ah && addend) && !(ep_mh && relu_src), PP_ERR_ARG,
               "pp_conv2d_nhwc_bwd_data_bf16x3: addend / relu_src given both as f32 and as planes");
  PP_CHECK_ARG(ctx, (!ep_ah || (ld_add >= d->cin && ld_add % 4 == 0)) && (!ep_mh || (ld_rs >= d->cin && ld_rs % 4 == 0)), PP_ERR_SHAPE,
               "pp_conv2d_nhwc_bwd_data_bf16x3: addend / relu_src planes");
  if (rc) return rc;
  PP_CHECK_ARG(ctx, !chi || (dy && !dy_hi && pp_is_packed(chi, clo)), PP_ERR_ARG, "pp_conv2d_nhwc_bwd_data_bf16x3: split capture needs the f32 operand");
  PP_CHECK_ARG(ctx, (dy || (dy_hi && dy_lo)) && w_hi && w_lo && (dx || (dx_hi && dx_lo)), PP_ERR_ARG, "pp_conv2d_nhwc_bwd_data_bf16x3: null tensor");
  PP_CHECK_ARG(ctx, (dy_hi == nullptr) == (dy_lo == nullptr) && d->ld_y % 8 == 0, PP_ERR_ARG, "pp_conv2d_nhwc_bwd_data_bf16x3: planes / ld_y");
  PP_CHECK_ARG(ctx, pp_is_packed(dy_hi, dy_lo) && pp_is_packed(dx_hi, dx_lo) && pp_is_packed(ep_ah, ep_al) && pp_is_aligned16(ep_mh), PP_ERR_ALIGN,
               "pp_conv2d_nhwc_bwd_data_bf16x3: planes must be packed (lo = hi + 16 bytes, 16-byte aligned)");
  PP_CHECK_ARG(ctx, (!dx_hi || (d->cin % 8 == 0 && d->ld_x % 8 == 0)) && (!ep_ah || ld_add % 8 == 0) && (!ep_mh || ld_rs % 8 == 0), PP_ERR_SHAPE,
               "pp_conv2d_nhwc_bwd_data_bf16x3: planes need channel counts and leading dimensions %% 8 == 0");
  const int cred = (d->cout + 31) / 32 * 32;
  PP_CHECK_ARG(ctx, d->cin % 16 == 0 && d->ld_y >= cred && d->ld_y % 4 == 0, PP_ERR_SHAPE,
               "pp_conv2d_nhwc_bwd_data_bf16x3: dy needs ld_y >= %d (cout rounded up to 32, zero padded)", cred);
  PP_CHECK_ARG(ctx, (!dy || pp_is_aligned16(dy)) && pp_is_aligned16(w_hi) && pp_is_aligned16(w_lo) && (!dx || pp_is_aligned16(dx)), PP_ERR_ALIGN,
               "pp_conv2d_nhwc_bwd_data_bf16x3: tensors must be 16-byte aligned");
  PP_CHECK_ARG(ctx, (!addend || (ld_add >= d->cin && ld_add % 4 == 0 && pp_is_aligned16(addend))) &&
                        (!relu_src || (ld_rs >= d->cin && ld_rs % 4 == 0 && pp_is_aligned16(relu_src))),
               PP_ERR_SHAPE, "pp_conv2d_nhwc_bwd_data_bf16x3: addend / relu_src");
  IgemmParams p;
  memset(&p, 0, sizeof(p));
  p.src = dy; p.out = dx; p.bias = nullptr; p.addend = addend; p.mask_src = relu_src;
  p.add_hi = ep_ah; p.add_lo = ep_al; p.mask_hi = ep_mh;
  p.ld_src = d->ld_y; p.ld_w = d->ld_w; p.ld_out = d->ld_x; p.ld_add = ld_add; p.ld_mask = ld_rs;
  p.relu = 0;
  p.n_seg = d->in.n_seg;
  fill_segs(ctx, d, false, p.seg, &p.M, &p.src_rows);
  p.Cred = cred; p.Nout = d->cin; p.w_tap_rows = d->cin;
  p.kh = d->kh; p.kw = d->kw;
  p.mul = 1; p.tsign = -1; p.off_y = d->pad_t; p.off_x = d->pad_l; p.div = d->stride;
  p.w_ty0 = 0; p.w_tx0 = 0; p.w_tstep = 1; p.w_kw = d->kw; p.w_taps = d->kh * d->kw;
  PP_CHECK_ARG(ctx, (dx_hi == nullptr) == (dx_lo == nullptr) && (!dx_hi || (d->ld_x % 4 == 0 && pp_is_aligned16(dx_hi) && pp_is_aligned16(dx_lo))),
               PP_ERR_ARG, "pp_conv2d_nhwc_bwd_data_bf16x3: output planes");
  static const bool s2_classes = []() { const char* e = getenv("PP_CONV3_S2CLASSES"); return !(e && e[0] == '0'); }();
  const bool all_f32 = dy && dx && !dy_hi && !dx_hi, all_planes = dy_hi && dx_hi && !dx;
  static const int rl_mode = []() { const char* e = getenv("PP_SPARSE_DGRAD"); return e ? atoi(e) : 22; }();
  bool rl_ok = skip_flags && skip_scratch_ok && rl_mode && (all_f32 || all_planes) && !chi && d->stride == 1 && d->kh == 3 && d->kw == 3 &&
               d->pad_t == 1 && d->pad_l == 1 && p.bias == nullptr && igemm3_fast_ok(p, all_planes, d->cin, cred / 8);
  for (int i = 0; i < p.n_seg && rl_ok; ++i)
    rl_ok = p.seg[i].OH == p.seg[i].SH && p.seg[i].OW == p.seg[i].SW && p.seg[i].row_begin == p.seg[i].src_row_begin;
  PP_CHECK_ARG(ctx, !lazy_in || rl_ok, PP_ERR_ARG,
               "pp_conv2d_nhwc_bwd_data_bf16x3: dy was declared lazy (unwritten outside its flagged blocks) but the listed-block launch "
               "does not apply to this call");
  if (skip_scratch_ok && !rl_ok)
    PP_HIP(ctx, hipMemsetAsync(const_cast<unsigned char*>(skip_flags) + (p.M + 31) / 32, 1, (size_t)((p.M + 31) / 32), ctx->stream));
  if (d->stride == 2 && s2_classes && (all_f32 || all_planes) && d->in.n_seg == 1) {
    IgemmParams q = p;
    q.div = 1;
    const int H = d->in.h[0], W = d->in.w[0];
    bool ok = true;
    IgemmParams cls[4];
    for (int c = 0; c < 4 && ok; ++c) {
      const int cy = c >> 1, cx = c & 1;
      IgemmParams& r = cls[c];
      r = q;
      const int ty0 = (cy + d->pad_t) & 1, tx0 = (cx + d->pad_l) & 1;
      r.kh = ty0 < d->kh ? (d->kh - ty0 + 1) / 2 : 0;
      r.kw = tx0 < d->kw ? (d->kw - tx0 + 1) / 2 : 0;
      r.off_y = (cy + d->pad_t - ty0) / 2;
      r.off_x = (cx + d->pad_l - tx0) / 2;
      r.w_ty0 = ty0; r.w_tx0 = tx0; r.w_tstep = 2; r.w_kw = d->kw;
      if (r.kh == 0 || r.kw == 0) r.kh = r.kw = 0;
      r.seg[0].OH = (H - cy + 1) / 2;
      r.seg[0].OW = (W - cx + 1) / 2;
      r.M = d->in.n_img * r.seg[0].OH * r.seg[0].OW;
      r.sc_on = 1; r.sc_H = H; r.sc_W = W; r.sc_cy = cy; r.sc_cx = cx;
      if (r.M > 0 && r.kh > 0 && !(igemm3_fast_ok(r, all_planes, d->cin, cred / 8) && r.M < (1 << 24))) ok = false;
    }
    if (ok) {
      if (chi) split_capture_pass(ctx->stream, p, chi, clo);
      for (int c = 0; c < 4; ++c) {
        if (cls[c].M <= 0) continue;
        if (cls[c].kh > 0) {
          dispatch3(ctx, cls[c], dy_hi, dy_lo, w_hi, w_lo, d->cin, cred / 8, dx_hi, dx_lo);
        } else {
          const long long total = (long long)cls[c].M * ((cls[c].Nout + 3) >> 2);
          long long blocks = (total + 255) / 256;
          const long long cap = (long long)(ctx->n_cu > 0 ? ctx->n_cu : 256) * 8;
          if (blocks > cap) blocks = cap;
          hipLaunchKernelGGL(class_fill_kernel, dim3((unsigned)blocks), dim3(256), 0, ctx->stream, cls[c], addend, relu_src, dx, dx_hi, dx_lo);
        }
      }
      PP_CHECK_LAUNCH(ctx, "pp_conv2d_nhwc_bwd_data_bf16x3");
      return PP_OK;
    }
  }
  if (rl_ok) {
    const int nb = (p.M + 31) / 32;
    unsigned char* out_flags = const_cast<unsigned char*>(skip_flags) + nb;
    int* out_list = const_cast<int*>(skip_list_in) + nb + 1;
    if (rl_mode == 22)
      launch_igemm3_rowlist<2, 2>(ctx->stream, p, dy_hi, dy_lo, w_hi, w_lo, d->cin, cred / 8, dx_hi, dx_lo, skip_flags, out_flags, out_list, ctx->ws,
                                  ctx->ws_bytes, !lazy_out);
    else
      launch_igemm3_rowlist<1, 2>(ctx->stream, p, dy_hi, dy_lo, w_hi, w_lo, d->cin, cred / 8, dx_hi, dx_lo, skip_flags, out_flags, out_list, ctx->ws,
                                  ctx->ws_bytes, !lazy_out);
    PP_CHECK_LAUNCH(ctx, "pp_conv2d_nhwc_bwd_data_bf16x3");
    return PP_OK;
  }
  dispatch3(ctx, p, dy_hi, dy_lo, w_hi, w_lo, d->cin, cred / 8, dx_hi, dx_lo, chi, clo, skip_flags);
  PP_CHECK_LAUNCH(ctx, "pp_conv2d_nhwc_bwd_data_bf16x3");
  return PP_OK;
}
namespace {

typedef short shortx4 __attribute__((ext_vector_type(4)));


template <int TM, int TN, bool AP>
__global__ __launch_bounds__(256, (TM * TN == 4) ? 2 : 3) void wgrad3_kernel(const Wgrad3Params p, const float* __restrict__ g_src,
                                                                            const float* __restrict__ g_dy,
                                                                            const uint4* __restrict__ g_xhi, const uint4* __restrict__ g_xlo,
                                                                            const uint4* __restrict__ g_dhi, const uint4* __restrict__ g_dlo,
                                                                            float* __restrict__ g_dw, float* __restrict__ g_dbias) {
  constexpr int BM = 64 * TM, BN = 64 * TN, BK = 32;
  constexpr int PA = BM + 32, PB = BN + 32;
  __shared__ __attribute__((aligned(16))) unsigned short smem[2 * BK * (PA + PB)];
  unsigned short* Xhi = smem;
  unsigned short* Xlo = Xhi + BK * PA;
  unsigned short* Ghi = Xlo + BK * PA;
  unsigned short* Glo = Ghi + BK * PB;

  const int tid = threadIdx.x, lane = tid & 63, wave = tid >> 6;
  const float inv_g = p.inv_scale ? *p.inv_scale : 1.f;
  const int wm = wave >> 1, wn = wave & 1;
  int b = xcd_remap((int)blockIdx.x, (int)gridDim.x);
  const int tile_n = b % p.n_tiles_n;
  b /= p.n_tiles_n;
  const int tile_k = b % p.n_tiles_k;
  const int split = b / p.n_tiles_k;
  const int tap = tile_k / p.k_tiles_per_tap;
  const int ci0 = (tile_k - tap * p.k_tiles_per_tap) * BM;
  const int ty = tap / p.kw, tx = tap - ty * p.kw;
  const int n0 = tile_n * BN;
  const int m_begin = split * p.rows_per_split;
  const int m_end = min(p.M, m_begin + p.rows_per_split);
  const int n_steps = (m_end - m_begin + BK - 1) / BK;

  const int prow = tid >> 3, q8 = tid & 7;
  constexpr int QA = BM / 32, QB = BN / 32;
  struct WRow { int m, n, y, x, seg_end, sb, OH, OW, SH, SW; } w;
  auto decode = [&](int m) {
    w.m = m;
    int rbeg = p.seg[0].row_begin;
    w.sb = p.seg[0].src_row_begin; w.OH = p.seg[0].OH; w.OW = p.seg[0].OW; w.SH = p.seg[0].SH; w.SW = p.seg[0].SW;
    w.seg_end = p.n_seg > 1 ? p.seg[1].row_begin : p.M;
    for (int s = 1; s < p.n_seg; ++s) {
      if (m >= p.seg[s].row_begin) {
        rbeg = p.seg[s].row_begin; w.sb = p.seg[s].src_row_begin; w.OH = p.seg[s].OH; w.OW = p.seg[s].OW;
        w.SH = p.seg[s].SH; w.SW = p.seg[s].SW;
        w.seg_end = (s + 1 < p.n_seg) ? p.seg[s + 1].row_begin : p.M;
      }
    }
    const int local = m < p.M ? m - rbeg : 0;
    const int hw = w.OH * w.OW;
    w.n = local / hw;
    const int rem = local - w.n * hw;
    w.y = rem / w.OW;
    w.x = rem - w.y * w.OW;
  };
  decode(m_begin + prow);

  constexpr int OA = (BM / 64 > 0) ? BM / 64 : 1, OB = (BN / 64 > 0) ? BN / 64 : 1;
  float4 ra[QA], rb[QB];
  uint4 pah[OA], pal[OA], pbh[OB], pbl[OB];
  float4 bsum[QB];
#pragma unroll
  for (int j = 0; j < QB; ++j) bsum[j] = make_float4(0.f, 0.f, 0.f, 0.f);
  const bool do_bias = (g_dbias != nullptr) && (tile_k == 0);

  auto load_step = [&]() {
    const int sy = w.y * p.stride + ty - p.pad_t;
    const int sx = w.x * p.stride + tx - p.pad_l;
    const bool in_rng = w.m < m_end;
    const bool ok = in_rng && ((unsigned)sy < (unsigned)w.SH) && ((unsigned)sx < (unsigned)w.SW);
    const long long xrow = (long long)(w.sb + w.n * w.SH * w.SW + sy * w.SW + sx) * p.ld_src + ci0;
    if (AP) {
#pragma unroll
      for (int j = 0; j < OA; ++j) {
        const long long o8 = 2 * ((xrow >> 3) + q8 + 8 * j);
        pah[j] = ok ? g_xhi[o8] : make_uint4(0u, 0u, 0u, 0u);
        pal[j] = ok ? g_xlo[o8] : make_uint4(0u, 0u, 0u, 0u);
      }
#pragma unroll
      for (int j = 0; j < OB; ++j) {
        const int c = n0 + 8 * (q8 + 8 * j);
        const bool okb = in_rng && c < p.ld_dy;
        const long long o8 = 2 * ((((long long)w.m * p.ld_dy + n0) >> 3) + q8 + 8 * j);
        pbh[j] = okb ? g_dhi[o8] : make_uint4(0u, 0u, 0u, 0u);
        pbl[j] = okb ? g_dlo[o8] : make_uint4(0u, 0u, 0u, 0u);
      }
    } else {
      const float* src = g_src + xrow;
#pragma unroll
      for (int j = 0; j < QA; ++j)
        ra[j] = ok ? *reinterpret_cast<const float4*>(src + 4 * (q8 + 8 * j)) : make_float4(0.f, 0.f, 0.f, 0.f);
      const float* dyr = g_dy + (long long)w.m * p.ld_dy + n0;
#pragma unroll
      for (int j = 0; j < QB; ++j) {
        const int c = n0 + 4 * (q8 + 8 * j);
        rb[j] = (in_rng && c < p.ld_dy) ? *reinterpret_cast<const float4*>(dyr + 4 * (q8 + 8 * j)) : make_float4(0.f, 0.f, 0.f, 0.f);
      }
    }
    const int m2 = w.m + BK;
    if (m2 >= w.seg_end) {
      decode(m2);
    } else {
      w.m = m2;
      w.x += BK;
      while (w.x >= w.OW) { w.x -= w.OW; ++w.y; }
      while (w.y >= w.OH) { w.y -= w.OH; ++w.n; }
    }
  };
  auto store_step = [&]() {
    if (AP) {
#pragma unroll
      for (int j = 0; j < OA; ++j) {
        const int off = prow * PA + 8 * (q8 + 8 * j);
        if (8 * (q8 + 8 * j) < BM) {
          *reinterpret_cast<uint4*>(Xhi + off) = pah[j];
          *reinterpret_cast<uint4*>(Xlo + off) = pal[j];
        }
      }
#pragma unroll
      for (int j = 0; j < OB; ++j) {
        const int off = prow * PB + 8 * (q8 + 8 * j);
        if (8 * (q8 + 8 * j) < BN) {
          *reinterpret_cast<uint4*>(Ghi + off) = pbh[j];
          *reinterpret_cast<uint4*>(Glo + off) = pbl[j];
          if (do_bias) {
            const unsigned int hw[4] = {pbh[j].x, pbh[j].y, pbh[j].z, pbh[j].w}, lw[4] = {pbl[j].x, pbl[j].y, pbl[j].z, pbl[j].w};
            float v[8];
#pragma unroll
            for (int e = 0; e < 4; ++e) fmt_value2(hw[e], lw[e], &v[2 * e], &v[2 * e + 1]);
            bsum[2 * j].x += v[0]; bsum[2 * j].y += v[1]; bsum[2 * j].z += v[2]; bsum[2 * j].w += v[3];
            bsum[2 * j + 1].x += v[4]; bsum[2 * j + 1].y += v[5]; bsum[2 * j + 1].z += v[6]; bsum[2 * j + 1].w += v[7];
          }
        }
      }
      return;
    }
#pragma unroll
    for (int j = 0; j < QA; ++j) {
      uint2 hi, lo;
      split4(ra[j], &hi, &lo);
      const int off = prow * PA + 4 * (q8 + 8 * j);
      *reinterpret_cast<uint2*>(Xhi + off) = hi;
      *reinterpret_cast<uint2*>(Xlo + off) = lo;
    }
#pragma unroll
    for (int j = 0; j < QB; ++j) {
      uint2 hi, lo;
      split4(rb[j], &hi, &lo);
      const int off = prow * PB + 4 * (q8 + 8 * j);
// ... 506 lines not shown
```

pyrapose_amd/csrc/ctx.hip:

```cpp
#include <stdlib.h>

#include "pp_internal.h"

extern "C" const char* pp_version(void) { return "pyrapose_hip 0.6 (gfx950; convolutions on packed planes in two formats -- bf16 pairs / bf16x3 and P16 / f16c8 (f16 + block-scaled e5m2 MFMA) -- and exact f32 MFMA; sparse 3D-box backward, pose tail, device augmentation)"; }

extern "C" int pp_ctx_create(pp_ctx** out, int device, void* hip_stream) {
  if (!out) return PP_ERR_ARG;
  *out = nullptr;
  int n_dev = 0;
  hipError_t e = hipGetDeviceCount(&n_dev);
  if (e != hipSuccess) return (int)e;
  if (device < 0 || device >= n_dev) return PP_ERR_ARG;
  pp_ctx* c = (pp_ctx*)calloc(1, sizeof(pp_ctx));
  if (!c) return PP_ERR_ARG;
  c->device = device;
  c->stream = (hipStream_t)hip_stream;
  hipDeviceProp_t prop;
  e = hipGetDeviceProperties(&prop, device);
  if (e != hipSuccess) {
    free(c);
    return (int)e;
  }
  c->n_cu = prop.multiProcessorCount;
  snprintf(c->name, sizeof(c->name), "%s (%s)", prop.name, prop.gcnArchName);
  c->err[0] = 0;
  *out = c;
  return PP_OK;
}

extern "C" void pp_ctx_destroy(pp_ctx* ctx) { free(ctx); }

extern "C" int pp_ctx_set_stream(pp_ctx* ctx, void* hip_stream) {
  PP_REQUIRE_CTX(ctx);
  ctx->stream = (hipStream_t)hip_stream;
  return PP_OK;
}

extern "C" int pp_ctx_set_workspace(pp_ctx* ctx, void* zeroed, size_t bytes) {
  PP_REQUIRE_CTX(ctx);
  PP_CHECK_ARG(ctx, (zeroed == nullptr) == (bytes == 0) && pp_is_aligned16(zeroed), PP_ERR_ARG, "pp_ctx_set_workspace: bad buffer");
  ctx->ws = (float*)zeroed;
  ctx->ws_bytes = bytes;
  return PP_OK;
}

extern "C" int pp_ctx_set_split_capture(pp_ctx* ctx, void* hi, void* lo) {
  PP_REQUIRE_CTX(ctx);
  PP_CHECK_ARG(ctx, (hi == nullptr) == (lo == nullptr) && pp_is_aligned16(hi) && pp_is_aligned16(lo), PP_ERR_ARG,
               "pp_ctx_set_split_capture: hi and lo go together, 16-byte aligned");
  ctx->cap_hi = hi;
  ctx->cap_lo = lo;
  return PP_OK;
}

extern "C" int pp_ctx_set_epilogue_planes(pp_ctx* ctx, const void* add_hi, const void* add_lo, const void* mask_hi) {
  PP_REQUIRE_CTX(ctx);
  PP_CHECK_ARG(ctx, (add_hi == nullptr) == (add_lo == nullptr), PP_ERR_ARG, "pp_ctx_set_epilogue_planes: add_hi and add_lo go together");
  PP_CHECK_ARG(ctx, pp_is_packed(add_hi, add_lo) && pp_is_aligned16(mask_hi), PP_ERR_ALIGN,
               "pp_ctx_set_epilogue_planes: planes must be packed (lo = hi + 16 bytes) and 16-byte aligned");
  ctx->ep_add_hi = add_hi;
  ctx->ep_add_lo = add_lo;
  ctx->ep_mask_hi = mask_hi;
  return PP_OK;
}

extern "C" int pp_ctx_set_row_block_skip(pp_ctx* ctx, const unsigned char* flags, const int* list) {
  PP_REQUIRE_CTX(ctx);
  ctx->skip_flags = flags;
  ctx->skip_list = list;
  return PP_OK;
}

extern "C" int pp_ctx_set_row_block_lazy(pp_ctx* ctx, int lazy_out, int lazy_in) {
  PP_REQUIRE_CTX(ctx);
  ctx->lazy_out = lazy_out != 0;
  ctx->lazy_in = lazy_in != 0;
  return PP_OK;
}

extern "C" int pp_ctx_set_row_block_out(pp_ctx* ctx, const unsigned char* flags, int* list) {
  PP_REQUIRE_CTX(ctx);
  PP_CHECK_ARG(ctx, (flags == nullptr) == (list == nullptr), PP_ERR_ARG, "pp_ctx_set_row_block_out: flags and list go together");
  ctx->out_flags = flags;
  ctx->out_list = list;
  return PP_OK;
}

extern "C" int pp_ctx_set_planes_format(pp_ctx* ctx, int fmt) {
  PP_REQUIRE_CTX(ctx);
  PP_CHECK_ARG(ctx, fmt == 0 || fmt == 1, PP_ERR_ARG, "pp_ctx_set_planes_format: 0 (bf16 pairs) or 1 (P16)");
  ctx->planes_fmt = fmt;
  return PP_OK;
}

extern "C" int pp_ctx_set_grad_scale(pp_ctx* ctx, const float* scale2_dev) {
  PP_REQUIRE_CTX(ctx);
  ctx->grad_scale = scale2_dev;
  return PP_OK;
}

extern "C" const char* pp_last_error_string(pp_ctx* ctx) { return ctx ? ctx->err : "no context"; }

extern "C" int pp_device_info(pp_ctx* ctx, int* n_cu, char* name, int name_len) {
  PP_REQUIRE_CTX(ctx);
  if (n_cu) *n_cu = ctx->n_cu;
  if (name && name_len > 0) {
    strncpy(name, ctx->name, (size_t)name_len - 1);
    name[name_len - 1] = 0;
  }
  return PP_OK;
}
```

pyrapose_amd/csrc/pp_internal.h:

```cpp
#pragma once
#include <hip/hip_runtime.h>
#include <stdarg.h>
#include <stdio.h>
#include <string.h>

#include "pyrapose_hip.h"

struct pp_ctx {
  int device;
  hipStream_t stream;
  int n_cu;
  char name[128];
  char err[512];
  float* ws;
  size_t ws_bytes;
  void* cap_hi;
  void* cap_lo;
  const void* ep_add_hi;
  const void* ep_add_lo;
  const void* ep_mask_hi;
  const int* skip_list;
  const unsigned char* skip_flags;
  int lazy_out, lazy_in;
  const unsigned char* out_flags;
  int* out_list;
  int planes_fmt;
  const float* grad_scale;
};

static inline int pp_fail(pp_ctx* ctx, int code, const char* fmt, ...) {
  if (ctx) {
    va_list ap;
    va_start(ap, fmt);
    vsnprintf(ctx->err, sizeof(ctx->err), fmt, ap);
    va_end(ap);
  }
  return code;
}

#define PP_REQUIRE_CTX(ctx) \
  do {                      \
    if (!(ctx)) return PP_ERR_NOCTX; \
  } while (0)

#define PP_CHECK_ARG(ctx, cond, code, ...)            \
  do {                                                \
    if (!(cond)) return pp_fail(ctx, code, __VA_ARGS__); \
  } while (0)

#define PP_CHECK_LAUNCH(ctx, what)                                                   \
  do {                                                                               \
    hipError_t e__ = hipGetLastError();                                              \
    if (e__ != hipSuccess)                                                           \
      return pp_fail(ctx, (int)e__, "%s: launch failed: %s", what, hipGetErrorString(e__)); \
  } while (0)

#define PP_HIP(ctx, call)                                                                        \
  do {                                                                                           \
    hipError_t e__ = (call);                                                                     \
    if (e__ != hipSuccess) return pp_fail(ctx, (int)e__, "%s: %s", #call, hipGetErrorString(e__)); \
  } while (0)

static inline long long pp_rowspace_rows(const pp_rowspace* rs) {
  long long r = 0;
  for (int s = 0; s < rs->n_seg; ++s) r += (long long)rs->n_img * rs->h[s] * rs->w[s];
  return r;
}

static inline int pp_rowspace_ok(const pp_rowspace* rs) {
  if (rs->n_img <= 0 || rs->n_seg <= 0 || rs->n_seg > PP_MAX_SEG) return 0;
  for (int s = 0; s < rs->n_seg; ++s)
    if (rs->h[s] <= 0 || rs->w[s] <= 0) return 0;
  return pp_rowspace_rows(rs) < (1ll << 31);
}

static inline int pp_is_aligned16(const void* p) { return (((uintptr_t)p) & 15u) == 0; }
static inline int pp_is_packed(const void* hi, const void* lo) {
  return (hi == nullptr && lo == nullptr) || (hi != nullptr && (const char*)lo == (const char*)hi + 16 && pp_is_aligned16(hi));
}
```

pyrapose_amd/engine.py:

```python
import os as _os
from collections import OrderedDict

import numpy as np
import torch

from . import arch, ops
from ._lib import ParamDesc, RowSpace


def _ru(v, m):
    return (v + m - 1) // m * m


def tf_same_pad(n_in, k, s):
    out = -(-n_in // s)
    total = max((out - 1) * s + k - n_in, 0)
    return total // 2


class Op(object):
    __slots__ = ("fn", "kind", "name", "flops", "wrange", "lane", "reads", "waits", "done_ev")

    def __init__(self, fn, kind, name="", flops=0.0, wrange=None, lane=0):
        self.fn, self.kind, self.name, self.flops, self.wrange, self.lane = fn, kind, name, flops, wrange, lane
# ... 599 lines not shown
    def _pyramid_buffer(self, level_shapes):
        B = self.B
        rows = [B * h * w for h, w in level_shapes]
        pyr_t = None if self.po else torch.empty((sum(rows), 256), dtype=torch.float32, device="cuda")
        cuts, r0 = [], 0
        for n in rows:
            cuts.append((r0, r0 + n))
            r0 += n
        sl = [pyr_t[a:b] if pyr_t is not None else None for a, b in cuts]
        pyr_pl = _new_planes(sum(rows), 256) if self.po else None
        spl = [(pyr_pl[0][a:b], pyr_pl[1][a:b]) if pyr_pl else None for a, b in cuts]
        return pyr_t, pyr_pl, rows, sl, spl

    def _build_sparse_fpn(self, C3, C4, C5):
        L3 = self._conv("fpn_lat3", C3)
        with self._on(1):
            L4 = self._conv("fpn_lat4", C4)
            L5 = self._conv("fpn_lat5", C5)
            S4 = self._upadd("fpn_sum4", L5, L4)
            M4 = self._conv("fpn_mid4", S4)
        S3 = self._upadd("fpn_sum3", L4, L3)
        M3 = self._conv("fpn_mid3", S3)
        D3 = self._conv("fpn_down3", M3)
        F3 = self._add("fpn_fin3", [M3, L3])
        lv = [L3.shapes[0], L4.shapes[0], L5.shapes[0]]
        pyr_t, pyr_pl, rows, sl, spl = self._pyramid_buffer(lv)
        P3 = self._conv("P3", F3, out_t=sl[0], out_pl=spl[0])
        with self._on(1):
            F4 = self._add("fpn_fin4", [D3, M4, L4])
            D4 = self._conv("fpn_down4", M4)
            P4 = self._conv("P4", F4, out_t=sl[1], out_pl=spl[1])
            F5 = self._add("fpn_fin5", [D4, L5])
            P5 = self._conv("P5", F5, out_t=sl[2], out_pl=spl[2])
        needs = self.train
        pyr = self._new_act("pyramid", lv, 256, 256, needs, False, pyr_t, pyr_pl, pyr_pl is not None, fmt=P3.fmt)
        pyr.producer = getattr(P3, "producer", None)
        pyr.prod_ops = [o for part in (P3, P4, P5) for o in part.prod_ops]
        self.graph_ops.append(dict(kind="alias", y=pyr, parts=[P3, P4, P5], rows=rows))
        return pyr, P3

    def _build_pyramid_features(self, C3, C4, C5):
        R5 = self._conv("C5_reduced", C5)
        R4 = self._conv("C4_reduced", C4)
        R3 = self._conv("C3_reduced", C3)
        S4 = self._upadd("td_sum4", R5, R4)
        S3 = self._upadd("td_sum3", S4, R3)
        lv = [R3.shapes[0], R4.shapes[0], R5.shapes[0]]
        if self.pyramid == "p3p7":
            s6 = (-(-R5.shapes[0][0] // 2), -(-R5.shapes[0][1] // 2))
            lv += [s6, (-(-s6[0] // 2), -(-s6[1] // 2))]
        pyr_t, pyr_pl, rows, sl, spl = self._pyramid_buffer(lv)
        P3 = self._conv("P3_con", S3, out_t=sl[0], out_pl=spl[0])
        P4 = self._conv("P4_con", S4, out_t=sl[1], out_pl=spl[1])
        P5 = self._conv("P5_con", R5, out_t=sl[2], out_pl=spl[2])
        parts = [P3, P4, P5]
        if self.pyramid == "p3p7":
            P6 = self._conv("P6_con", C5, out_t=sl[3], out_pl=spl[3])
            R6 = self._relu("P6_relu", P6)
            P7 = self._conv("P7_con", R6, out_t=sl[4], out_pl=spl[4])
            parts += [P6, P7]
        pyr = self._new_act("pyramid", lv, 256, 256, self.train, False, pyr_t, pyr_pl, pyr_pl is not None, fmt=P3.fmt)
        pyr.producer = getattr(P3, "producer", None)
        pyr.prod_ops = [o for part in parts for o in part.prod_ops]
        self.graph_ops.append(dict(kind="alias", y=pyr, parts=parts, rows=rows))
        return pyr, P3

    def _relu(self, name, x):
        out = self._new_act(name, x.shapes, x.C, x.ld, x.needs_grad, True, planes=self.po, fmt=x.fmt)
        lane = self._lane
        ctx = self.ctxs[lane].twin(x.fmt)
        vx, vo = x.view(), out.view()
        self._push(Op(lambda: ops.relu_fwd_v(ctx, vx, vo), "pointwise", name, lane=lane), (x,), out)
        self.graph_ops.append(dict(kind="relu", y=out, x=x))
        return out

    def _upadd(self, name, src, other):
        (sh, sw), (th, tw) = src.shapes[0], other.shapes[0]
        other = self._convert(other, src.fmt)
        out = self._new_act(name, [(th, tw)], src.C, src.ld, src.needs_grad or other.needs_grad, planes=self.po, fmt=src.fmt)
        lane, B = self._lane, self.B
        ctx = self.ctxs[lane].twin(src.fmt)
        vs, vt, vo = src.view(), other.view(), out.view()
        self._push(Op(lambda: ops.upsample_add_fwd_v(ctx, B, sh, sw, th, tw, src.C, vs, vt, vo), "pointwise", name, lane=lane),
                   (src, other), out)
        self.graph_ops.append(dict(kind="upadd", y=out, src=src, other=other))
        return out

    def _add(self, name, ins):
        ins = [ins[0]] + [self._convert(i, ins[0].fmt) for i in ins[1:]]
        out = self._new_act(name, ins[0].shapes, ins[0].C, ins[0].ld, any(i.needs_grad for i in ins), planes=self.po, fmt=ins[0].fmt)
        lane = self._lane
        ctx = self.ctxs[lane].twin(ins[0].fmt)
        va, vb, vc = ins[0].view(), ins[1].view(), (ins[2].view() if len(ins) > 2 else None)
        vo = out.view()
        self._push(Op(lambda: ops.add_n_v(ctx, va, vb, vc, vo), "pointwise", name, lane=lane), ins, out)
        self.graph_ops.append(dict(kind="add", y=out, ins=ins))
        return out

    def _new_grad(self, rows, ld, fmt=0):
        if self.po and ld % 8 == 0:
            g = Grad(None, _new_planes(rows, ld), fmt)
            self._plane_grads.append(g)
            return g
        return Grad(torch.empty((rows, ld), dtype=torch.float32, device="cuda"))

    def _finalize(self, act, producer=None):
        ctx = self.ctx.twin(act.fmt)
        grads = [c[1] for c in act.contribs if c[0] in ("tensor", "masked")]
        dgrads = [c for c in act.contribs if c[0] == "dgrad"]
        if any(c[0] == "masked" for c in act.contribs):
            assert len(act.contribs) == 1, act.name
            return grads[0]
        if not grads and not dgrads:
            return None
        acc = None
        if len(grads) == 1:
            acc = grads[0]
        elif len(grads) > 1:
            acc = self._new_grad(act.rows, act.ld, act.fmt)
            srcs, rest = grads[:3], grads[3:]
            while True:
                va, vb, vc = srcs[0].view(), (srcs[1].view() if len(srcs) > 1 else None), (srcs[2].view() if len(srcs) > 2 else None)
                vo = ops.tview(acc.t, acc.pl)
                self.bwd_ops.append(Op(lambda va=va, vb=vb, vc=vc, vo=vo: ops.add_n_v(ctx, va, vb, vc, vo), "pointwise", "add:" + act.name))
                if not rest:
                    break
                srcs, rest = [acc] + rest[:2], rest[2:]
        if act.relu and not dgrads:
            raise NotImplementedError("relu output %s without a data-gradient consumer" % act.name)
        if not dgrads:
            return acc
        for i, (_, op, gy) in enumerate(dgrads):
            last = i == len(dgrads) - 1
            mask = act if (act.relu and last) else None
            pl = op.get("planes")
            if pl is not None and pl["dg_hi"] is not None:
                gcap = op.get("g_cap")
                sk = op.get("skip")
                in_place = (sk is not None and i > 0 and mask is None and acc is not None and gcap is None
                            and _os.environ.get("PP_SPARSE_INPLACE", "1") != "0")
                out = acc if in_place else self._new_grad(act.rows, act.ld, act.fmt)
                lazy_out = (sk is not None and len(dgrads) == 1 and acc is None and gcap is None and gy.pl is not None and out.pl is not None
                            and self._lazy_reader(producer) and _os.environ.get("PP_SPARSE_WITHIN", "1") != "0"
                            and _os.environ.get("PP_SPARSE_LAZY", "1") != "0" and _os.environ.get("PP_SPARSE_DGRAD", "22") != "0")
                lazy_in = bool(gy.lazy)
                dy_t, dy_pl = (None, gy.pl) if gy.pl is not None else (gy.t, None)
                a_t = a_pl = m_t = m_hi = None
                if acc is not None:
                    a_t, a_pl = (acc.t, None) if acc.t is not None else (None, acc.pl)
                if mask is not None:
                    m_t, m_hi = (mask.t, None) if mask.t is not None else (None, mask.pl[0])
                if gcap is not None:
                    assert dy_t is not None
                self.bwd_ops.append(Op(lambda d=op["desc"], dy_t=dy_t, dy_pl=dy_pl, dh=pl["dg_hi"], dl=pl["dg_lo"], a_t=a_t, a_pl=a_pl, m_t=m_t,
                                       m_hi=m_hi, out=out, gcap=gcap, sk=sk, lazy_out=lazy_out, lazy_in=lazy_in:
                                       ops.conv_bwd_data3(ctx, d, dy_t, dh, dl, a_t, m_t, out.t, dy_pl, out.pl, gcap, sk, a_pl, m_hi,
                                                          lazy_out=lazy_out, lazy_in=lazy_in), "conv_dgrad",
                                       op["spec"].name, op["flops"]))
                out.within = sk[0][sk[0].numel() // 2:] if (sk is not None and acc is None and _os.environ.get("PP_SPARSE_WITHIN", "1") != "0") else None
                out.lazy = lazy_out
                assert not lazy_out or out.within is not None
                pw = op.pop("pending_wgrad", None)
                if pw is not None:
                    self.bwd_ops.append(pw)
            else:
                assert gy.t is not None and (acc is None or acc.t is not None) and (mask is None or mask.t is not None), act.name
                out = Grad(torch.empty((act.rows, act.ld), dtype=torch.float32, device="cuda"))
                self.bwd_ops.append(Op(lambda d=op["desc"], gy=gy, w=op["w"], a=(acc.t if acc is not None else None),
                                       m=(mask.t if mask is not None else None), out=out:
                                       ops.conv_bwd_data(ctx, d, gy.t, w, a, m, out.t), "conv_dgrad", op["spec"].name, op["flops"]))
            acc = out
        return acc

    def _lazy_reader(self, producer):
        if producer is None or producer.get("kind") != "conv" or producer.get("residual") is not None:
            return False
        s_, pl_, x_, y_ = producer["spec"], producer.get("planes"), producer["x"], producer["y"]
        geo = (_os.environ.get("PP_CONV3_FAST", "1") != "0" and min(h * w for h, w in x_.shapes) >= 32 and x_.rows < (1 << 24)
               and x_.rows * x_.ld * 4 < (1 << 31) and y_.rows * y_.ld * 4 < (1 << 31) and list(x_.shapes) == list(y_.shapes))
        return self._sparse_layer(s_) and pl_ is not None and pl_["dg_hi"] is not None and x_.pl is not None and y_.pl is not None and geo

    def _build_backward(self):
        ctx, P = self.ctx, self.params
        f32 = dict(dtype=torch.float32, device="cuda")
        self.g_reg = torch.zeros((self.reg_out.rows, self.reg_out.ld), **f32)
        self.g_cls = torch.zeros((self.cls_out.rows, self.cls_out.ld), **f32)
        self.g_mask = torch.zeros((self.mask_out.rows, self.mask_out.ld), **f32)
        for out, gt in ((self.reg_out, self.g_reg), (self.cls_out, self.g_cls), (self.mask_out, self.g_mask)):
            g = Grad(gt, None, out.fmt)
            if self.po and out.ld % 8 == 0:
                g.pl = _new_planes(out.rows, out.ld)
                sctx, sc = ctx.twin(out.fmt), (self.gscale if out.fmt == 1 else None)
                self.bwd_ops.append(Op(lambda gt=gt, pl=g.pl, sctx=sctx, sc=sc: ops.split_planes3(sctx, gt, pl[0], pl[1], sc), "pointwise",
                                       "split:" + out.name))
            out.contribs.append(("tensor", g))
        for op in reversed(self.graph_ops):
            kind = op["kind"]
            if kind == "stop":
                break
            y = op["y"]
            if not y.needs_grad:
                continue
            g = self._finalize(y, op)
            if g is None:
                continue
            if kind == "convert":
                x = op["x"]
                if x.needs_grad:
                    gx = self._new_grad(x.rows, x.ld, x.fmt)
                    assert g.pl is not None and gx.pl is not None, x.name
                    sc, idx = (self.gscale, 1) if (g.fmt == 1 and x.fmt == 0) else ((self.gscale, 0) if (g.fmt == 0 and x.fmt == 1) else (None, 0))
                    lone = x.relu and not any(o is not op and o.get("kind") == "conv" and o.get("x") is x for o in self.graph_ops)
                    mhi = x.pl[0] if lone else None
                    self.bwd_ops.append(Op(lambda g=g, gx=gx, sc=sc, idx=idx, mhi=mhi: ops.convert_planes(ctx, g.pl, g.fmt, gx.pl, gx.fmt, sc, idx, mhi),
                                           "pointwise", "convert_bwd:" + x.name))
                    x.contribs.append(("masked" if lone else "tensor", gx))
                continue
            if kind == "conv":
                s, x = op["spec"], op["x"]
                lctx = ctx.twin(y.fmt)
                if self._sparse_layer(s) and g.contiguous() and len(g.shape()) == 2:
                    nb = (g.shape()[0] + 31) // 32
                    skip = op["skip"] = (torch.zeros((2 * nb,), dtype=torch.uint8, device="cuda"),
                                         torch.zeros((2 * (nb + 1),), dtype=torch.int32, device="cuda"))
                    cols = min((y.C + 3) // 4 * 4, g.shape()[1])
                    if g.t is not None:
                        self.bwd_ops.append(Op(lambda gt=g.t, cols=cols, skip=skip, lctx=lctx: ops.row_block_list(lctx, gt, cols, skip[0], skip[1]),
                                               "pointwise", "rowblocks:" + s.name))
                    else:
                        self.bwd_ops.append(Op(lambda gp=g.pl, cols=cols, skip=skip, within=g.within, lctx=lctx:
                                               ops.row_block_list_planes(lctx, gp, cols, skip[0], skip[1], within),
                                               "pointwise", "rowblocks:" + s.name))
                if s.trainable:
                    dw = P.view(P.grad, s.name + "/kernel")
                    db = P.view(P.grad, s.name + "/bias") if s.bias else None
                    ek = P.entries[s.name + "/kernel"]
                    eb = P.entries[s.name + "/bias"]
                    wr = (ek["offset"], eb["offset"] + eb["count"])
                    wl = 1 % self.n_lanes
                    wctx = self.ctxs[wl].twin(y.fmt)
                    pl_ = op.get("planes")
                    if (op.get("x_cap") is not None and x.needs_grad and pl_ is not None and pl_["dg_hi"] is not None
                            and g.pl is None and g.t.shape == (y.rows, y.ld) and g.t.is_contiguous()):
                        gc = op["g_cap"] = _new_planes(y.rows, y.ld)
                        fn = lambda d=op["desc"], x=x, g=g, dw=dw, db=db, wctx=wctx, xp=op["x_cap"], gp=gc: \
                            ops.conv_bwd_weight3(wctx, d, x.t, g.t, dw, db, xp, gp)
                        op["pending_wgrad"] = Op(fn, "conv_wgrad", s.name, op["flops"], wr, wl)
                        fn = None
                    elif self.conv_mode == "bf16x3" and s.cin % 64 == 0:
                        both = x.pl is not None and g.pl is not None
                        assert both or (x.t is not None and g.t is not None), "weight gradient of %s: operands in different formats" % s.name
                        sk = op.get("skip")
                        assert not g.lazy or (both and sk is not None), s.name
                        fn = lambda d=op["desc"], xt=(None if both else x.t), gt=(None if both else g.t), dw=dw, db=db, wctx=wctx, \
                            xp=(x.pl if both else None), gp=(g.pl if both else None), sk=sk, lz=g.lazy: \
                            ops.conv_bwd_weight3(wctx, d, xt, gt, dw, db, xp, gp, sk, lazy_in=lz)
                    else:
                        assert x.t is not None and g.t is not None, s.name
                        fn = lambda d=op["desc"], xt=x.t, g=g, dw=dw, db=db, wctx=wctx: ops.conv_bwd_weight(wctx, d, xt, g.t, dw, db)
                    if fn is not None:
                        self.bwd_ops.append(Op(fn, "conv_wgrad", s.name, op["flops"], wr, wl))
                if x.needs_grad:
                    x.contribs.append(("dgrad", op, g))
                r = op["residual"]
                if r is not None and r.needs_grad:
                    r.contribs.append(("tensor", g))
            elif kind == "add":
                for i in op["ins"]:
                    if i.needs_grad:
                        i.contribs.append(("tensor", g))
            elif kind == "upadd":
                src, other = op["src"], op["other"]
                if other.needs_grad:
                    other.contribs.append(("tensor", g))
                if src.needs_grad:
                    gs = self._new_grad(src.rows, src.ld, src.fmt)
                    (sh, sw), (th, tw) = src.shapes[0], other.shapes[0]
                    vg, vs = g.view(), ops.tview(gs.t, gs.pl)
                    uctx = ctx.twin(src.fmt)
                    self.bwd_ops.append(Op(lambda vg=vg, vs=vs, sh=sh, sw=sw, th=th, tw=tw, c=src.C, uctx=uctx:
                                           ops.upsample_add_bwd_v(uctx, self.B, sh, sw, th, tw, c, vg, None, vs), "pointwise", "upbwd:" + src.name))
                    src.contribs.append(("tensor", gs))
            elif kind == "relu":
                if op["x"].needs_grad:
                    op["x"].contribs.append(("tensor", g))
            elif kind == "alias":
                r0 = 0
                for part, n in zip(op["parts"], op["rows"]):
                    part.contribs.append(("tensor", g.rows(r0, r0 + n)))
                    r0 += n
        left = [op["spec"].name for op in self.graph_ops if op.get("pending_wgrad") is not None]
        assert not left, "weight gradients waiting for a bwd-data launch that never came: %s" % left

    def _fork(self, lanes):
        if self.n_lanes == 1:
            return
        ev = torch.cuda.Event()
        ev.record(self.streams[0])
        for l in lanes:
            self.streams[l].wait_event(ev)

    def _join(self, lanes):
        for l in lanes:
            ev = torch.cuda.Event()
            ev.record(self.streams[l])
            self.streams[0].wait_event(ev)

    RESIDENT = "resident"

    def _load_input(self, inp, lane):
        if inp[0] == "f32":
            if inp[1] is not None:
                with torch.cuda.stream(self.streams[lane]):
                    self.x_in.copy_(inp[1])
            return
        x4 = self.acts["input4"]
        xd = inp[1]
        with torch.cuda.stream(self.streams[lane]):
            if len(inp) > 3 and inp[3] is not None:
                xd = ops.warp_affine_u8(self.ctxs[lane], xd, inp[3], "linear", inp[4], inp[5])
            if self.stem3:
                ops.preprocess_caffe_u8_padded(self.ctxs[lane], xd, inp[2], x4.t, *self.stem_frame)
            else:
                ops.preprocess_caffe_u8(self.ctxs[lane], xd, inp[2], x4.t)

    @staticmethod
    def _input_key(inp):
        return (inp[0], Engine.RESIDENT if inp[1] is None else inp[1])

    @staticmethod
    def _same_input(a, b):
        return a is not None and a[0] == b[0] and a[1] is b[1]

    def _run_fwd_ops(self, lo, hi, skip_pack):
        streams = self.streams
        for i in range(lo, hi):
            op = self.fwd_ops[i]
            st = streams[op.lane]
            for ev in op.waits:
                st.wait_event(ev)
            if not (skip_pack and i == 0):
                op.fn()
            if op.done_ev is not None:
                op.done_ev.record(st)

    def _forward(self, inp, nxt):
        cur = self._enter()
        lp, ne = self.prefix_lane, self.n_prefix_early
        assert self.fwd_ops[0].name == "pack_rgb"
        pre, self._prefetched = self._prefetched, None
        start = 0
        if lp is not None and self._same_input(pre, self._input_key(inp)):
            start = ne
        else:
            if lp is not None:
                self._fork([lp])
            self._load_input(inp, lp if lp is not None else 0)
        trig = self.pf_trigger if (lp is not None and nxt is not None) else ne + 1
        self._run_fwd_ops(start, trig if lp is not None else len(self.fwd_ops), inp[0] == "u8")
        if lp is not None:
            if nxt is not None:
                ev = torch.cuda.Event()
                ev.record(self.streams[0])
                self.streams[lp].wait_event(ev)
                nxt = ("f32", None) if nxt[1] is Engine.RESIDENT else nxt
                self._load_input(nxt, lp)
                self._run_fwd_ops(0, ne, nxt[0] == "u8")
                self._prefetched = self._input_key(nxt)
            self._run_fwd_ops(trig, len(self.fwd_ops), False)
        self._join(list(range(1, self.n_lanes)))
        self._leave(cur)

    def forward(self, x=None, next_x=None):
        self._forward(("f32", x), None if next_x is None else ("f32", next_x))
# ... 189 lines not shown
```

pyrapose_amd/ops.py:

```python
import ctypes as C

import numpy as np
import torch

from ._lib import ConvDesc, ParamDesc, RowSpace, TView, check, lib


def _ptr(t):
    if t is None:
        return None
    assert t.is_cuda, "pyrapose_amd ops need device tensors"
    return C.c_void_p(t.data_ptr())


class Context:

    def __init__(self, device=0, stream=None):
        if not torch.cuda.is_available():
            raise RuntimeError("pyrapose_amd: no GPU visible (torch.cuda.is_available() is False); "
                               "the HIP path has no CPU fallback")
        self.device = int(device)
        torch.cuda.set_device(self.device)
        self.handle = C.c_void_p()
        s = stream if stream is not None else torch.cuda.current_stream(self.device)
# ... 127 lines not shown

def planes_to_f32(planes, fmt=0):
    hi, lo = planes
    rows = hi.shape[0]
    if fmt == 0:
        return (hi.contiguous().view(torch.bfloat16).float() + lo.contiguous().view(torch.bfloat16).float()).reshape(rows, -1)
    rem = (lo.contiguous().to(torch.int32) & 0xff00).to(torch.int16).view(torch.float16).float() / 4096.0
    return (hi.contiguous().view(torch.float16).float() + rem).reshape(rows, -1)


def weight_planes_to_f32(hi, lo, fmt=0):
    if fmt == 0:
        return hi.contiguous().view(torch.bfloat16).float() + lo.contiguous().view(torch.bfloat16).float()
    rem = ((lo.contiguous().to(torch.int32) & 0xff) << 8).to(torch.int16).view(torch.float16).float() / 4096.0
    return hi.contiguous().view(torch.float16).float() + rem


def split_planes3(ctx, src, hi, lo, scale=None):
    if scale is None:
        check(lib.pp_split_planes_bf16x3(ctx.handle, src.numel(), _ptr(src), _ptr(hi), _ptr(lo)), ctx.handle, "pp_split_planes_bf16x3")
    else:
        check(lib.pp_split_planes_scaled_bf16x3(ctx.handle, src.numel(), _ptr(src), _ptr(hi), _ptr(lo), _ptr(scale)), ctx.handle,
              "pp_split_planes_scaled_bf16x3")


def grad_scale_from_counts(ctx, counts, scale2, log2_adjust=0):
    check(lib.pp_grad_scale_from_counts_adj(ctx.handle, _ptr(counts), int(counts.numel()), _ptr(scale2), int(log2_adjust)), ctx.handle,
          "pp_grad_scale_from_counts")


def set_grad_scale(ctx, scale2):
    ctx._grad_scale_keep = scale2
    check(lib.pp_ctx_set_grad_scale(ctx.handle, _ptr(scale2)), ctx.handle, "pp_ctx_set_grad_scale")


def _set_capture(ctx, planes):
    if planes is not None:
        check(lib.pp_ctx_set_split_capture(ctx.handle, _ptr(planes[0]), _ptr(planes[1])), ctx.handle, "pp_ctx_set_split_capture")


def row_block_list(ctx, x, cols, flags=None, blocks=None):
    rows, ld = x.shape
    nb = (rows + 31) // 32
    if flags is None:
        flags = torch.zeros((2 * nb,), dtype=torch.uint8, device=x.device)
    if blocks is None:
        blocks = torch.zeros((2 * (nb + 1),), dtype=torch.int32, device=x.device)
    check(lib.pp_row_block_list(ctx.handle, _ptr(x), rows, x.stride(0), int(cols), _ptr(flags), _ptr(blocks)), ctx.handle, "pp_row_block_list")
    return flags, blocks


def row_block_list_planes(ctx, planes, cols, flags, blocks, within=None):
    hi, lo = planes
    rows = hi.shape[0]
    if within is not None:
        assert within.dtype == torch.uint8 and within.is_contiguous() and within.numel() >= (rows + 31) // 32
        check(lib.pp_row_block_list_planes_within(ctx.handle, _ptr(hi), _ptr(lo), rows, planes_ld(planes), int(cols), _ptr(within), _ptr(flags),
                                                  _ptr(blocks)), ctx.handle, "pp_row_block_list_planes_within")
    else:
        check(lib.pp_row_block_list_planes(ctx.handle, _ptr(hi), _ptr(lo), rows, planes_ld(planes), int(cols), _ptr(flags), _ptr(blocks)),
              ctx.handle, "pp_row_block_list_planes")
    return flags, blocks


def _set_epilogue_planes(ctx, add_planes, mask_hi):
    if add_planes is not None or mask_hi is not None:
        ah, al = add_planes if add_planes is not None else (None, None)
        check(lib.pp_ctx_set_epilogue_planes(ctx.handle, _ptr(ah), _ptr(al), _ptr(mask_hi)), ctx.handle, "pp_ctx_set_epilogue_planes")


def tview(t=None, planes=None):
    v = TView()
    v.f32 = t.data_ptr() if t is not None else None
    v.hi = planes[0].data_ptr() if planes is not None else None
    v.lo = planes[1].data_ptr() if planes is not None else None
    v._keep = (t, planes)
    return v


def _numel(v):
    t, planes = v._keep
    return (t if t is not None else planes[0]).numel()


def add_n_v(ctx, a, b, c, out):
    null = TView()
    check(lib.pp_add_n_v(ctx.handle, _numel(a), C.byref(a), C.byref(b if b is not None else null), C.byref(c if c is not None else null),
                         C.byref(out)), ctx.handle, "pp_add_n_v")


def relu_fwd_v(ctx, x, y):
    check(lib.pp_relu_fwd_v(ctx.handle, _numel(x), C.byref(x), C.byref(y)), ctx.handle, "pp_relu_fwd_v")


def upsample_add_fwd_v(ctx, n_img, sh, sw, th, tw, c, src, other, out):
    null = TView()
    check(lib.pp_upsample_nearest_add_fwd_v(ctx.handle, n_img, sh, sw, th, tw, c, C.byref(src), C.byref(other if other is not None else null),
                                            C.byref(out)), ctx.handle, "pp_upsample_nearest_add_fwd_v")


def upsample_add_bwd_v(ctx, n_img, sh, sw, th, tw, c, dtarget, base, dsrc):
    null = TView()
    check(lib.pp_upsample_nearest_add_bwd_v(ctx.handle, n_img, sh, sw, th, tw, c, C.byref(dtarget), C.byref(base if base is not None else null),
                                            C.byref(dsrc)), ctx.handle, "pp_upsample_nearest_add_bwd_v")


def merge_planes3(ctx, planes, dst):
    check(lib.pp_merge_planes_bf16x3(ctx.handle, dst.numel(), _ptr(planes[0]), _ptr(planes[1]), _ptr(dst)), ctx.handle, "pp_merge_planes_bf16x3")


def planes_stats(ctx, planes, cols, stats, within=None):
    hi, lo = planes
    check(lib.pp_planes_stats(ctx.handle, _ptr(hi), _ptr(lo), int(hi.shape[0]), planes_ld(planes), int(cols), _ptr(within), _ptr(stats)), ctx.handle,
          "pp_planes_stats")
    return stats


def positive_row_blocks(ctx, rs, n_anchor, y_true, flags):
    check(lib.pp_positive_row_blocks(ctx.handle, C.byref(rs), int(n_anchor), int(y_true.shape[-1]), _ptr(y_true), _ptr(flags)), ctx.handle,
          "pp_positive_row_blocks")
    return flags


def row_block_dilate(ctx, d, in_flags, out_flags):
    check(lib.pp_row_block_dilate(ctx.handle, C.byref(d), _ptr(in_flags), _ptr(out_flags)), ctx.handle, "pp_row_block_dilate")
    return out_flags


def set_row_block_out(ctx, flags, blocks):
    check(lib.pp_ctx_set_row_block_out(ctx.handle, _ptr(flags), _ptr(blocks)), ctx.handle, "pp_ctx_set_row_block_out")


def _set_skip(ctx, skip, lazy_out=False, lazy_in=False):
    if skip is not None:
        check(lib.pp_ctx_set_row_block_skip(ctx.handle, _ptr(skip[0]), _ptr(skip[1])), ctx.handle, "pp_ctx_set_row_block_skip")
    if lazy_out or lazy_in:
        if skip is None:
            raise ValueError("lazy sparse gradients go with a row-block skip hint (dy_skip)")
        check(lib.pp_ctx_set_row_block_lazy(ctx.handle, int(bool(lazy_out)), int(bool(lazy_in))), ctx.handle, "pp_ctx_set_row_block_lazy")


def conv_fwd3(ctx, d, x, w_hi, w_lo, bias, residual, relu, y, x_planes=None, y_planes=None, x_capture=None, res_planes=None):
    _set_capture(ctx, x_capture)
    _set_epilogue_planes(ctx, res_planes, None)
    ld_res = residual.stride(0) if residual is not None else (planes_ld(res_planes) if res_planes is not None else 0)
    xh, xl = x_planes if x_planes is not None else (None, None)
    yh, yl = y_planes if y_planes is not None else (None, None)
    check(lib.pp_conv2d_nhwc_fwd_bf16x3(ctx.handle, C.byref(d), _ptr(x), _ptr(xh), _ptr(xl), _ptr(w_hi), _ptr(w_lo), _ptr(bias),
                                        _ptr(residual), ld_res, int(bool(relu)), _ptr(y), _ptr(yh), _ptr(yl)), ctx.handle,
          "pp_conv2d_nhwc_fwd_bf16x3")


def conv_bwd_data3(ctx, d, dy, w_hi, w_lo, addend, relu_src, dx, dy_planes=None, dx_planes=None, dy_capture=None, dy_skip=None,
                   addend_planes=None, relu_src_hi=None, lazy_out=False, lazy_in=False):
    _set_capture(ctx, dy_capture)
    _set_skip(ctx, dy_skip, lazy_out, lazy_in)
    _set_epilogue_planes(ctx, addend_planes, relu_src_hi)
    ld_add = addend.stride(0) if addend is not None else (planes_ld(addend_planes) if addend_planes is not None else 0)
    ld_rs = relu_src.stride(0) if relu_src is not None else (relu_src_hi.stride(0) // 2 if relu_src_hi is not None else 0)
    dh, dl = dy_planes if dy_planes is not None else (None, None)
    xh, xl = dx_planes if dx_planes is not None else (None, None)
    check(lib.pp_conv2d_nhwc_bwd_data_bf16x3(ctx.handle, C.byref(d), _ptr(dy), _ptr(dh), _ptr(dl), _ptr(w_hi), _ptr(w_lo), _ptr(addend),
                                             ld_add, _ptr(relu_src), ld_rs, _ptr(dx), _ptr(xh), _ptr(xl)), ctx.handle,
          "pp_conv2d_nhwc_bwd_data_bf16x3")


def conv_bwd_weight3(ctx, d, x, dy, dw, dbias, x_planes=None, dy_planes=None, dy_skip=None, lazy_in=False):
    _set_skip(ctx, dy_skip, False, lazy_in)
    xh, xl = x_planes if x_planes is not None else (None, None)
    dh, dl = dy_planes if dy_planes is not None else (None, None)
    check(lib.pp_conv2d_nhwc_bwd_weight_bf16x3(ctx.handle, C.byref(d), _ptr(x), _ptr(dy), _ptr(xh), _ptr(xl), _ptr(dh), _ptr(dl),
                                               _ptr(dw), _ptr(dbias)), ctx.handle, "pp_conv2d_nhwc_bwd_weight_bf16x3")


def maxpool3x3s2(ctx, n_img, h, w, c, x, oh, ow, y):
    check(lib.pp_maxpool3x3s2_fwd(ctx.handle, n_img, h, w, c, _ptr(x), oh, ow, _ptr(y)), ctx.handle, "pp_maxpool3x3s2_fwd")


def upsample_add_fwd(ctx, n_img, sh, sw, th, tw, c, src, other, out):
    check(lib.pp_upsample_nearest_add_fwd(ctx.handle, n_img, sh, sw, th, tw, c, _ptr(src), _ptr(other), _ptr(out)),
          ctx.handle, "pp_upsample_nearest_add_fwd")


def upsample_add_bwd(ctx, n_img, sh, sw, th, tw, c, dtarget, base, dsrc):
    check(lib.pp_upsample_nearest_add_bwd(ctx.handle, n_img, sh, sw, th, tw, c, _ptr(dtarget), _ptr(base), _ptr(dsrc)),
          ctx.handle, "pp_upsample_nearest_add_bwd")


def add_n(ctx, a, b, c, out):
    check(lib.pp_add_n(ctx.handle, a.numel(), _ptr(a), _ptr(b), _ptr(c), _ptr(out)), ctx.handle, "pp_add_n")


def relu_fwd(ctx, x, y):
    check(lib.pp_relu_fwd(ctx.handle, x.numel(), _ptr(x), _ptr(y)), ctx.handle, "pp_relu_fwd")


def warp_affine_u8(ctx, images_u8, matrices, interpolation="linear", border="replicate", cval=0, out=None):
    B, H, W = images_u8.shape[:3]
    ch = images_u8.shape[3] if images_u8.dim() == 4 else 1
    m = np.ascontiguousarray(np.asarray(matrices, np.float64).reshape(B, -1)[:, :6])
    if out is None:
        out = torch.empty_like(images_u8)
    check(lib.pp_warp_affine_u8(ctx.handle, B, H, W, ch, m.ctypes.data_as(C.POINTER(C.c_double)), {"nearest": 0, "linear": 1}[interpolation],
                                {"constant": 0, "replicate": 1}[border], int(cval), _ptr(images_u8), _ptr(out)), ctx.handle, "pp_warp_affine_u8")
    return out


def resize_scale(rows, cols, min_side=480, max_side=640):
    s = C.c_double(0)
    check(lib.pp_resize_scale(int(rows), int(cols), int(min_side), int(max_side), C.byref(s)), None, "pp_resize_scale")
    return s.value


def resize_linear_u8(ctx, images_u8, scale):
    B, H, W = images_u8.shape[:3]
    ch = images_u8.shape[3] if images_u8.dim() == 4 else 1
    dh, dw = int(np.rint(H * scale)), int(np.rint(W * scale))
    out = torch.empty((B, dh, dw) + ((ch,) if images_u8.dim() == 4 else ()), dtype=torch.uint8, device=images_u8.device)
    check(lib.pp_resize_linear_u8(ctx.handle, B, H, W, ch, float(scale), dh, dw, _ptr(images_u8), _ptr(out)), ctx.handle, "pp_resize_linear_u8")
    return out


def preprocess_caffe_u8(ctx, images_u8, sizes_hw, x4):
    Bn, H, W, _ = images_u8.shape
    assert images_u8.dtype == torch.uint8 and images_u8.is_contiguous()
    arr = (C.c_int * (2 * Bn))(*[int(v) for hw in sizes_hw for v in hw])
    check(lib.pp_preprocess_caffe_u8(ctx.handle, Bn, H, W, arr, _ptr(images_u8), _ptr(x4)), ctx.handle, "pp_preprocess_caffe_u8")


def pack_rgb_to_4_padded(ctx, x3, x4p, Hp, Wp, pad=3):
    Bn, H, W, _ = x3.shape
    check(lib.pp_pack_rgb_to_4_padded(ctx.handle, Bn, H, W, Hp, Wp, pad, _ptr(x3), _ptr(x4p)), ctx.handle, "pp_pack_rgb_to_4_padded")


def preprocess_caffe_u8_padded(ctx, images_u8, sizes_hw, x4p, Hp, Wp, pad=3):
    Bn, H, W, _ = images_u8.shape
    assert images_u8.dtype == torch.uint8 and images_u8.is_contiguous()
    arr = (C.c_int * (2 * Bn))(*[int(v) for hw in sizes_hw for v in hw])
    check(lib.pp_preprocess_caffe_u8_padded(ctx.handle, Bn, H, W, Hp, Wp, pad, arr, _ptr(images_u8), _ptr(x4p)), ctx.handle,
          "pp_preprocess_caffe_u8_padded")


def stem7x7s2_fwd3(ctx, n_img, H, W, Hp, Wp, x4p, w_hi, w_lo, cout, bias, relu, y):
    check(lib.pp_stem7x7s2_fwd_bf16x3(ctx.handle, n_img, H, W, Hp, Wp, _ptr(x4p), _ptr(w_hi), _ptr(w_lo), cout, _ptr(bias), int(bool(relu)),
                                      _ptr(y), y.stride(0)), ctx.handle, "pp_stem7x7s2_fwd_bf16x3")


def pack_rgb_to_4(ctx, x3, x4):
    check(lib.pp_pack_rgb_to_4(ctx.handle, x3.numel() // 3, _ptr(x3), _ptr(x4)), ctx.handle, "pp_pack_rgb_to_4")


def export_head(ctx, rs, n_anchor, n_val, src, apply_sigmoid, out):
    check(lib.pp_export_head(ctx.handle, C.byref(rs), n_anchor, n_val, _ptr(src), src.stride(0), int(apply_sigmoid), _ptr(out)),
          ctx.handle, "pp_export_head")


def count_positives(ctx, y_box, y_cls, y_mask, counts):
    rb = y_box.shape[0] * y_box.shape[1] if y_box is not None else 0
    rc = y_cls.shape[0] * y_cls.shape[1] if y_cls is not None else 0
    rm = y_mask.shape[0] * y_mask.shape[1] if y_mask is not None else 0
    cc = y_cls.shape[2] - 1 if y_cls is not None else 0
    cm = y_mask.shape[2] - 1 if y_mask is not None else 0
    check(lib.pp_count_positives(ctx.handle, rb, _ptr(y_box), rc, cc, _ptr(y_cls), rm, cm, _ptr(y_mask), _ptr(counts)),
          ctx.handle, "pp_count_positives")


def focal(ctx, rs, n_anchor, n_class, logits, y_true, alpha, gamma, count, loss_weight, loss_sum, dlogits):
    check(lib.pp_sigmoid_focal_fwd_bwd(ctx.handle, C.byref(rs), n_anchor, n_class, _ptr(logits), logits.stride(0),
                                       _ptr(y_true), alpha, gamma, _ptr(count), loss_weight, _ptr(loss_sum), _ptr(dlogits)),
          ctx.handle, "pp_sigmoid_focal_fwd_bwd")


def orth_l1(ctx, rs, n_anchor, pred, y_true, weight, sigma, count, loss_weight, loss_sum, dpred):
    check(lib.pp_orth_smoothl1_fwd_bwd(ctx.handle, C.byref(rs), n_anchor, _ptr(pred), pred.stride(0), _ptr(y_true), weight,
                                       sigma, _ptr(count), loss_weight, _ptr(loss_sum), _ptr(dpred)),
          ctx.handle, "pp_orth_smoothl1_fwd_bwd")


class Optimizer:
    def __init__(self, ctx, descs, total):
        arr = (ParamDesc * len(descs))(*descs)
        self.handle = C.c_void_p()
        self.ctx = ctx
        check(lib.pp_optimizer_create(ctx.handle, C.byref(self.handle), arr, len(descs), total), ctx.handle,
              "pp_optimizer_create")

    def grad_norm(self, w_master, g_eff, scales, gnorm_sq, l2_loss=None):
        check(lib.pp_grad_global_norm(self.ctx.handle, self.handle, _ptr(w_master), _ptr(g_eff), _ptr(scales),
                                      _ptr(gnorm_sq), _ptr(l2_loss)), self.ctx.handle, "pp_grad_global_norm")

    def adam_step(self, w_master, w_eff, g_eff, scales, m, v, gnorm_sq, lr, beta1, beta2, eps, clipnorm, step):
        check(lib.pp_adam_step_clipnorm(self.ctx.handle, self.handle, _ptr(w_master), _ptr(w_eff), _ptr(g_eff), _ptr(scales),
                                        _ptr(m), _ptr(v), _ptr(gnorm_sq), lr, beta1, beta2, eps, clipnorm, int(step)),
              self.ctx.handle, "pp_adam_step_clipnorm")

    def close(self):
        if self.handle:
            lib.pp_optimizer_destroy(self.handle)
            self.handle = C.c_void_p()


def _iarr(v):
    return (C.c_int * len(v))(*[int(x) for x in v])


def generate_base_anchors(base_size, ratios, scales):
    r = np.ascontiguousarray(ratios, np.float32)
# ... 298 lines not shown
```

Before: 603.3.

## Fuse next-layer row-block flag generation into sparse dgrad finish and parallelize compaction

The sparse dgrad split-K finish now runs a wider 8-channel kernel that also records, per 32-row block, whether the produced dx planes are nonzero. This lets the next layer's skip flags and list be built in the same pass instead of by a separate scan of dx. The single-block compaction kernel is replaced by a multi-block prefix kernel that fuses dilation and compaction. A legacy env switch keeps the old path. The cost is added complexity, more alignment preconditions and more per-op setup when building the engine.

```diff
diff --git a/include/pyrapose_hip.h b/include/pyrapose_hip.h
--- a/include/pyrapose_hip.h
+++ b/include/pyrapose_hip.h
@@ -32,6 +32,7 @@
 int pp_ctx_set_epilogue_planes(pp_ctx* ctx, const void* add_hi, const void* add_lo, const void* mask_hi);
 int pp_ctx_set_row_block_skip(pp_ctx* ctx, const unsigned char* flags, const int* list);
 int pp_ctx_set_row_block_lazy(pp_ctx* ctx, int lazy_out, int lazy_in);
+int pp_ctx_set_row_block_flags_out(pp_ctx* ctx, unsigned char* flags, int* list, int cols);
 const char* pp_last_error_string(pp_ctx* ctx);
 const char* pp_version(void);
 int pp_device_info(pp_ctx* ctx, int* n_cu, char* name_host, int name_len);
diff --git a/pyrapose_amd/_lib.py b/pyrapose_amd/_lib.py
--- a/pyrapose_amd/_lib.py
+++ b/pyrapose_amd/_lib.py
@@ -98,6 +98,7 @@
     "pp_ctx_set_row_block_skip": (_i, [_p, _p, _p]),
     "pp_ctx_set_row_block_out": (_i, [_p, _p, _p]),
     "pp_ctx_set_row_block_lazy": (_i, [_p, _i, _i]),
+    "pp_ctx_set_row_block_flags_out": (_i, [_p, _p, _p, _i]),
     "pp_positive_row_blocks": (_i, [_p, _p, _i, _i, _p, _p]),
     "pp_row_block_dilate": (_i, [_p, _p, _p, _p]),
     "pp_row_block_list_planes": (_i, [_p, _p, _p, _i, _i, _i, _p, _p]),
diff --git a/pyrapose_amd/csrc/conv3.hip b/pyrapose_amd/csrc/conv3.hip
--- a/pyrapose_amd/csrc/conv3.hip
+++ b/pyrapose_amd/csrc/conv3.hip
@@ -840,6 +840,88 @@
   }
 }
 
+__device__ __forceinline__ bool finish8(const IgemmParams& p, float4 a, float4 b, long long mo, int co, const float* __restrict__ g_addend,
+                                        const float* __restrict__ g_mask, float* __restrict__ g_out, void* __restrict__ g_ohi) {
+  if (p.add_hi) {
+    const uint4* q = reinterpret_cast<const uint4*>(p.add_hi) + 2 * ((mo * p.ld_add + co) >> 3);
+    const uint4 h = q[0], l = q[1];
+    float4 x, y;
+    fmt_value2(h.x, l.x, &x.x, &x.y);
+    fmt_value2(h.y, l.y, &x.z, &x.w);
+    fmt_value2(h.z, l.z, &y.x, &y.y);
+    fmt_value2(h.w, l.w, &y.z, &y.w);
+    a.x += x.x; a.y += x.y; a.z += x.z; a.w += x.w;
+    b.x += y.x; b.y += y.y; b.z += y.z; b.w += y.w;
+  } else if (g_addend) {
+    const float4 x = *reinterpret_cast<const float4*>(g_addend + mo * p.ld_add + co), y = *reinterpret_cast<const float4*>(g_addend + mo * p.ld_add + co + 4);
+    a.x += x.x; a.y += x.y; a.z += x.z; a.w += x.w;
+    b.x += y.x; b.y += y.y; b.z += y.z; b.w += y.w;
+  }
+  if (p.mask_hi) {
+    const uint4 k = reinterpret_cast<const uint4*>(p.mask_hi)[2 * ((mo * p.ld_mask + co) >> 3)];
+    a.x = fmt_pos(k.x & 0xffffu) ? a.x : 0.f; a.y = fmt_pos(k.x >> 16) ? a.y : 0.f; a.z = fmt_pos(k.y & 0xffffu) ? a.z : 0.f; a.w = fmt_pos(k.y >> 16) ? a.w : 0.f;
+    b.x = fmt_pos(k.z & 0xffffu) ? b.x : 0.f; b.y = fmt_pos(k.z >> 16) ? b.y : 0.f; b.z = fmt_pos(k.w & 0xffffu) ? b.z : 0.f; b.w = fmt_pos(k.w >> 16) ? b.w : 0.f;
+  } else if (g_mask) {
+    const float4 k = *reinterpret_cast<const float4*>(g_mask + mo * p.ld_mask + co), k2 = *reinterpret_cast<const float4*>(g_mask + mo * p.ld_mask + co + 4);
+    a.x = k.x > 0.f ? a.x : 0.f; a.y = k.y > 0.f ? a.y : 0.f; a.z = k.z > 0.f ? a.z : 0.f; a.w = k.w > 0.f ? a.w : 0.f;
+    b.x = k2.x > 0.f ? b.x : 0.f; b.y = k2.y > 0.f ? b.y : 0.f; b.z = k2.z > 0.f ? b.z : 0.f; b.w = k2.w > 0.f ? b.w : 0.f;
+  }
+  if (p.relu) {
+    a.x = fmaxf(a.x, 0.f); a.y = fmaxf(a.y, 0.f); a.z = fmaxf(a.z, 0.f); a.w = fmaxf(a.w, 0.f);
+    b.x = fmaxf(b.x, 0.f); b.y = fmaxf(b.y, 0.f); b.z = fmaxf(b.z, 0.f); b.w = fmaxf(b.w, 0.f);
+  }
+  if (g_out) {
+    *reinterpret_cast<float4*>(g_out + mo * p.ld_out + co) = a;
+    *reinterpret_cast<float4*>(g_out + mo * p.ld_out + co + 4) = b;
+  }
+  if (g_ohi) {
+    uint4 h, l;
+    split8(a, b, &h, &l);
+    uint4* dst = reinterpret_cast<uint4*>(g_ohi) + 2 * ((mo * p.ld_out + co) >> 3);
+    dst[0] = h;
+    dst[1] = l;
+    return fmt_any_nonzero(h.x | h.y | h.z | h.w, l.x | l.y | l.z | l.w);
+  }
+  return false;
+}
+
+__global__ __launch_bounds__(256) void rl_finish8_kernel(const IgemmParams p, int splits, const float* __restrict__ ws, const int* __restrict__ g_rl,
+                                                         const float* __restrict__ g_bias, const float* __restrict__ g_addend,
+                                                         const float* __restrict__ g_mask, float* __restrict__ g_out, void* __restrict__ g_ohi,
+                                                         unsigned char* __restrict__ next_flags) {
+  const int j = (int)(blockIdx.x >> 2);
+  if (j >= g_rl[0]) return;
+  bool any = false;
+  const int n8 = p.Nout >> 3;
+  const long long slice = (((long long)p.M + 31) & ~31ll) * p.ld_out;
+  const int m0 = g_rl[1 + j] * 32;
+  const int tx = threadIdx.x & 63, r0 = (int)((blockIdx.x & 3) << 3) + (int)(threadIdx.x >> 6);
+#pragma unroll
+  for (int rr = 0; rr < 2; ++rr) {
+    const int r = r0 + 4 * rr;
+    if (m0 + r >= p.M) break;
+    for (int c = tx; c < n8; c += 64) {
+      const int co = 8 * c;
+      const float* w = ws + ((long long)j * 32 + r) * p.ld_out + co;
+      float4 a = *reinterpret_cast<const float4*>(w), b = *reinterpret_cast<const float4*>(w + 4);
+      for (int s = 1; s < splits; ++s) {
+        const float4 q = *reinterpret_cast<const float4*>(w + s * slice), q2 = *reinterpret_cast<const float4*>(w + s * slice + 4);
+        a.x += q.x; a.y += q.y; a.z += q.z; a.w += q.w;
+        b.x += q2.x; b.y += q2.y; b.z += q2.z; b.w += q2.w;
+      }
+      if (g_bias) {
+        const float4 q = *reinterpret_cast<const float4*>(g_bias + co), q2 = *reinterpret_cast<const float4*>(g_bias + co + 4);
+        a.x += q.x; a.y += q.y; a.z += q.z; a.w += q.w;
+        b.x += q2.x; b.y += q2.y; b.z += q2.z; b.w += q2.w;
+      }
+      any |= finish8(p, a, b, (long long)(m0 + r), co, g_addend, g_mask, g_out, g_ohi);
+    }
+  }
+  if (next_flags) {
+    if (__syncthreads_or(any ? 1 : 0) && threadIdx.x == 0) next_flags[m0 >> 5] = 1;
+  }
+}
+
 __global__ void split_planes_kernel(size_t n8, const float4* __restrict__ src, uint4* __restrict__ hi, uint4* __restrict__ lo,
                                     const float* __restrict__ scale) {
   const float sc = scale ? *scale : 1.f;
@@ -922,6 +1004,56 @@
   if (tid == 0) list[0] = base;
 }
 
+__device__ __forceinline__ int rl_dilate_one(const IgemmParams& p, const unsigned char* __restrict__ in_flags, int b) {
+  const int r_lo = 32 * b, r_hi = min(32 * b + 31, p.M - 1);
+  int any = 0;
+  for (int s = 0; s < p.n_seg; ++s) {
+    const int seg_lo = p.seg[s].row_begin, seg_hi = (s + 1 < p.n_seg ? p.seg[s + 1].row_begin : p.M) - 1;
+    if (r_hi < seg_lo || r_lo > seg_hi) continue;
+    const int W = p.seg[s].OW;
+    for (int j = -1; j <= 1; ++j) {
+      int lo = r_lo - 1 + j * W, hi = r_hi + 1 + j * W;
+      lo = lo < 0 ? 0 : lo;
+      hi = hi > p.M - 1 ? p.M - 1 : hi;
+      for (int q = lo >> 5; q <= (hi >> 5); ++q) any |= in_flags[q];
+    }
+  }
+  return any ? 1 : 0;
+}
+
+__global__ __launch_bounds__(256) void rl_prep_kernel(const IgemmParams p, const unsigned char* __restrict__ in_flags, unsigned char* out_flags,
+                                                      int n_blocks, int* __restrict__ list, unsigned char* __restrict__ zero_flags) {
+  __shared__ int wave_cnt[4];
+  const int tid = threadIdx.x, lane = tid & 63, wave = tid >> 6;
+  const int c0 = (int)blockIdx.x * 256;
+  if (zero_flags && c0 + tid < n_blocks) zero_flags[c0 + tid] = 0;
+  int base = 0;
+  for (int i0 = 0; i0 < c0; i0 += 256)
+    base += __syncthreads_count(in_flags ? rl_dilate_one(p, in_flags, i0 + tid) : (out_flags[i0 + tid] != 0));
+  const int i = c0 + tid;
+  const bool f = i < n_blocks && (in_flags ? rl_dilate_one(p, in_flags, i) != 0 : out_flags[i] != 0);
+  if (in_flags && i < n_blocks) out_flags[i] = f ? 1 : 0;
+  const unsigned long long m = __ballot(f);
+  const int before = __popcll(m & ((1ull << lane) - 1ull));
+  if (lane == 0) wave_cnt[wave] = __popcll(m);
+  __syncthreads();
+  int off = base;
+  for (int w = 0; w < wave; ++w) off += wave_cnt[w];
+  if (f) list[1 + off + before] = i;
+  if (tid == 0 && blockIdx.x == gridDim.x - 1) list[0] = base + wave_cnt[0] + wave_cnt[1] + wave_cnt[2] + wave_cnt[3];
+}
+
+static void launch_row_block_compact(const pp_ctx* ctx, const unsigned char* flags, int nb, int* list) {
+  if (ctx->sparse_chain_legacy) {
+    hipLaunchKernelGGL(row_block_compact_kernel, dim3(1), dim3(256), 0, ctx->stream, flags, nb, list);
+  } else {
+    IgemmParams p;
+    memset(&p, 0, sizeof(p));
+    hipLaunchKernelGGL(rl_prep_kernel, dim3((unsigned)((nb + 255) / 256)), dim3(256), 0, ctx->stream, p, (const unsigned char*)nullptr,
+                       const_cast<unsigned char*>(flags), nb, list, (unsigned char*)nullptr);
+  }
+}
+
 }
 extern "C" int PP_API(pp_row_block_list)(pp_ctx* ctx, const float* x, int rows, int ld, int cols, unsigned char* flags, int* list) {
   PP_REQUIRE_CTX(ctx);
@@ -930,7 +1062,7 @@
   const int nb = (rows + 31) / 32, cols4 = (cols + 3) / 4;
   PP_CHECK_ARG(ctx, 4 * cols4 <= ld, PP_ERR_SHAPE, "pp_row_block_list: cols rounded up to 4 exceed ld");
   hipLaunchKernelGGL(row_block_flags_kernel, dim3((unsigned)nb), dim3(256), 0, ctx->stream, x, rows, ld, cols4, flags);
-  hipLaunchKernelGGL(row_block_compact_kernel, dim3(1), dim3(256), 0, ctx->stream, (const unsigned char*)flags, nb, list);
+  launch_row_block_compact(ctx, flags, nb, list);
   PP_CHECK_LAUNCH(ctx, "pp_row_block_list");
   return PP_OK;
 }
@@ -957,7 +1089,7 @@
   PP_CHECK_ARG(ctx, 4 * cols4 <= ld, PP_ERR_SHAPE, "pp_row_block_list_planes: cols rounded up to 4 exceed ld");
   hipLaunchKernelGGL(row_block_flags_planes_kernel, dim3((unsigned)nb), dim3(256), 0, ctx->stream, (const uint2*)x_hi, (const uint2*)x_lo, rows,
                      ld / 4, cols4, flags, within);
-  hipLaunchKernelGGL(row_block_compact_kernel, dim3(1), dim3(256), 0, ctx->stream, (const unsigned char*)flags, nb, list);
+  launch_row_block_compact(ctx, flags, nb, list);
   PP_CHECK_LAUNCH(ctx, "pp_row_block_list_planes");
   return PP_OK;
 }
@@ -1110,20 +1242,7 @@
                                  int n_blocks) {
   const int b = blockIdx.x * blockDim.x + threadIdx.x;
   if (b >= n_blocks) return;
-  const int r_lo = 32 * b, r_hi = min(32 * b + 31, p.M - 1);
-  int any = 0;
-  for (int s = 0; s < p.n_seg; ++s) {
-    const int seg_lo = p.seg[s].row_begin, seg_hi = (s + 1 < p.n_seg ? p.seg[s + 1].row_begin : p.M) - 1;
-    if (r_hi < seg_lo || r_lo > seg_hi) continue;
-    const int W = p.seg[s].OW;
-    for (int j = -1; j <= 1; ++j) {
-      int lo = r_lo - 1 + j * W, hi = r_hi + 1 + j * W;
-      lo = lo < 0 ? 0 : lo;
-      hi = hi > p.M - 1 ? p.M - 1 : hi;
-      for (int q = lo >> 5; q <= (hi >> 5); ++q) any |= in_flags[q];
-    }
-  }
-  out_flags[b] = any ? 1 : 0;
+  out_flags[b] = (unsigned char)rl_dilate_one(p, in_flags, b);
 }
 
 __global__ void rl_fill_kernel(const IgemmParams p, const unsigned char* __restrict__ live, const float* __restrict__ g_addend,
@@ -1185,7 +1304,8 @@
 template <int TM, int TN>
 static void launch_igemm3_rowlist(hipStream_t st, IgemmParams& p, const void* ahi, const void* alo, const void* whi, const void* wlo, int w_rows,
                                   int w_ld8, void* ohi, void* olo, const unsigned char* dy_flags, unsigned char* out_flags, int* out_list,
-                                  float* ws, size_t ws_bytes, bool fill = true) {
+                                  float* ws, size_t ws_bytes, bool fill = true, bool legacy = false, unsigned char* next_flags = nullptr,
+                                  int* next_list = nullptr, int next_cols = 0, bool* next_done = nullptr) {
   constexpr int BM = 64 * TM, BN = 64 * TN;
   const int nb = (p.M + 31) / 32;
   static const int want_splits = []() { const char* e = getenv("PP_SPARSE_DGRAD_SPLITS"); return e ? atoi(e) : 2; }();
@@ -1196,8 +1316,18 @@
     splits = want_splits;
     while (splits > 1 && (n_steps / splits < 24 || slice_bytes * splits > (long long)ws_bytes)) --splits;
   }
-  if (dy_flags) hipLaunchKernelGGL(rl_dilate_kernel, dim3((unsigned)((nb + 255) / 256)), dim3(256), 0, st, p, dy_flags, out_flags, nb);
-  hipLaunchKernelGGL(row_block_compact_kernel, dim3(1), dim3(256), 0, st, (const unsigned char*)out_flags, nb, out_list);
+  const bool finish8_ok = !legacy && p.Nout % 8 == 0 && (!ohi || (p.ld_out % 8 == 0 && (const char*)olo == (const char*)ohi + 16)) &&
+                          (!p.add_hi || (p.ld_add % 8 == 0 && (const char*)p.add_lo == (const char*)p.add_hi + 16)) &&
+                          (!p.mask_hi || p.ld_mask % 8 == 0);
+  const bool fuse_next = next_flags && next_list && splits > 1 && finish8_ok && ohi && next_cols == p.Nout;
+  if (next_done) *next_done = fuse_next;
+  if (legacy) {
+    if (dy_flags) hipLaunchKernelGGL(rl_dilate_kernel, dim3((unsigned)((nb + 255) / 256)), dim3(256), 0, st, p, dy_flags, out_flags, nb);
+    hipLaunchKernelGGL(row_block_compact_kernel, dim3(1), dim3(256), 0, st, (const unsigned char*)out_flags, nb, out_list);
+  } else {
+    hipLaunchKernelGGL(rl_prep_kernel, dim3((unsigned)((nb + 255) / 256)), dim3(256), 0, st, p, dy_flags, out_flags, nb, out_list,
+                       fuse_next ? next_flags : (unsigned char*)nullptr);
+  }
   p.n_tiles_n = (p.Nout + BN - 1) / BN;
   const int n_tiles_m = (nb + BM / 32 - 1) / (BM / 32);
   const long long a_bytes = p.src_rows * (long long)p.ld_src * 4, w_bytes = (long long)p.w_taps * w_rows * w_ld8 * 16;
@@ -1214,12 +1344,18 @@
     hipLaunchKernelGGL((igemm3f_kernel<TM, TN, false, false, false, true>), grid, dim3(256), 0, st, p, (const void*)p.src, nullptr,
                        (unsigned)a_bytes, whi, wlo, (unsigned)w_bytes, p.bias, p.addend, p.mask_src, p.out, (uint2*)nullptr, (uint2*)nullptr,
                        w_rows, w_ld8, splits, splits > 1 ? ws : (float*)nullptr, (const int*)out_list, dy_flags);
-  if (splits > 1)
+  if (splits > 1 && finish8_ok)
+    hipLaunchKernelGGL(rl_finish8_kernel, dim3((unsigned)(4 * nb)), dim3(256), 0, st, p, splits, (const float*)ws, (const int*)out_list, p.bias,
+                       p.addend, p.mask_src, p.out, ohi, fuse_next ? next_flags : (unsigned char*)nullptr);
+  else if (splits > 1)
     hipLaunchKernelGGL(rl_splitk_finish_kernel, dim3((unsigned)nb), dim3(256), 0, st, p, splits, (const float*)ws, (const int*)out_list, p.bias,
                        p.addend, p.mask_src, p.out, ohi, olo);
   const bool in_place = (ohi != nullptr && p.add_hi == (const void*)ohi && p.ld_add == p.ld_out && !p.out && !p.addend && !p.mask_hi &&
                          !p.mask_src && !p.relu) ||
                         (p.out != nullptr && p.addend == p.out && p.ld_add == p.ld_out && !ohi && !p.add_hi && !p.mask_hi && !p.mask_src && !p.relu);
+  if (fuse_next)
+    hipLaunchKernelGGL(rl_prep_kernel, dim3((unsigned)((nb + 255) / 256)), dim3(256), 0, st, p, (const unsigned char*)nullptr, next_flags, nb, next_list,
+                       (unsigned char*)nullptr);
   if (fill && !in_place)
     hipLaunchKernelGGL(rl_fill_kernel, dim3((unsigned)nb), dim3(256), 0, st, p, (const unsigned char*)out_flags, p.addend, p.mask_src, p.out, ohi,
                        olo);
@@ -1535,7 +1671,7 @@
       ok = p.seg[i].OH == p.seg[i].SH && p.seg[i].OW == p.seg[i].SW && p.seg[i].row_begin == p.seg[i].src_row_begin;
     PP_CHECK_ARG(ctx, ok, PP_ERR_SHAPE, "pp_conv2d_nhwc_fwd_bf16x3: the row-block-out hint needs a 3x3 stride-1 'same' conv on plane-stored input");
     launch_igemm3_rowlist<2, 2>(ctx->stream, p, x_hi, x_lo, w_hi, w_lo, d->cout, d->cin / 8, y_hi, y_lo, nullptr, const_cast<unsigned char*>(out_flags),
-                                out_list, ctx->ws, ctx->ws_bytes, false);
+                                out_list, ctx->ws, ctx->ws_bytes, false, ctx->sparse_chain_legacy != 0);
     PP_CHECK_LAUNCH(ctx, "pp_conv2d_nhwc_fwd_bf16x3");
     return PP_OK;
   }
@@ -1609,6 +1745,11 @@
   ctx->skip_list = nullptr;
   const bool lazy_out = ctx->lazy_out != 0, lazy_in = ctx->lazy_in != 0;
   ctx->lazy_out = ctx->lazy_in = 0;
+  unsigned char* next_flags = ctx->next_flags;
+  int* next_list = ctx->next_list;
+  const int next_cols = ctx->next_cols;
+  ctx->next_flags = nullptr;
+  ctx->next_list = nullptr;
   const void *ep_ah = ctx->ep_add_hi, *ep_al = ctx->ep_add_lo, *ep_mh = ctx->ep_mask_hi;
   ctx->ep_add_hi = ctx->ep_add_lo = ctx->ep_mask_hi = nullptr;
   int rc = check_desc(ctx, d, "pp_conv2d_nhwc_bwd_data_bf16x3");
@@ -1620,6 +1761,8 @@
   PP_CHECK_ARG(ctx, !chi || (dy && !dy_hi && pp_is_packed(chi, clo)), PP_ERR_ARG, "pp_conv2d_nhwc_bwd_data_bf16x3: split capture needs the f32 operand");
   PP_CHECK_ARG(ctx, (dy || (dy_hi && dy_lo)) && w_hi && w_lo && (dx || (dx_hi && dx_lo)), PP_ERR_ARG, "pp_conv2d_nhwc_bwd_data_bf16x3: null tensor");
   PP_CHECK_ARG(ctx, (dy_hi == nullptr) == (dy_lo == nullptr) && d->ld_y % 8 == 0, PP_ERR_ARG, "pp_conv2d_nhwc_bwd_data_bf16x3: planes / ld_y");
+  PP_CHECK_ARG(ctx, !next_flags || (dx_hi && dx_lo && next_cols <= d->ld_x), PP_ERR_ARG,
+               "pp_conv2d_nhwc_bwd_data_bf16x3: the row-block hint of dx (pp_ctx_set_row_block_flags_out) needs dx as planes");
   PP_CHECK_ARG(ctx, pp_is_packed(dy_hi, dy_lo) && pp_is_packed(dx_hi, dx_lo) && pp_is_packed(ep_ah, ep_al) && pp_is_aligned16(ep_mh), PP_ERR_ALIGN,
                "pp_conv2d_nhwc_bwd_data_bf16x3: planes must be packed (lo = hi + 16 bytes, 16-byte aligned)");
   PP_CHECK_ARG(ctx, (!dx_hi || (d->cin % 8 == 0 && d->ld_x % 8 == 0)) && (!ep_ah || ld_add % 8 == 0) && (!ep_mh || ld_rs % 8 == 0), PP_ERR_SHAPE,
@@ -1696,6 +1839,7 @@
         }
       }
       PP_CHECK_LAUNCH(ctx, "pp_conv2d_nhwc_bwd_data_bf16x3");
+      if (next_flags) return PP_API(pp_row_block_list_planes_within)(ctx, dx_hi, dx_lo, p.M, d->ld_x, next_cols, nullptr, next_flags, next_list);
       return PP_OK;
     }
   }
@@ -1703,17 +1847,22 @@
     const int nb = (p.M + 31) / 32;
     unsigned char* out_flags = const_cast<unsigned char*>(skip_flags) + nb;
     int* out_list = const_cast<int*>(skip_list_in) + nb + 1;
+    bool next_done = false;
     if (rl_mode == 22)
       launch_igemm3_rowlist<2, 2>(ctx->stream, p, dy_hi, dy_lo, w_hi, w_lo, d->cin, cred / 8, dx_hi, dx_lo, skip_flags, out_flags, out_list, ctx->ws,
-                                  ctx->ws_bytes, !lazy_out);
+                                  ctx->ws_bytes, !lazy_out, ctx->sparse_chain_legacy != 0, next_flags, next_list, next_cols, &next_done);
     else
       launch_igemm3_rowlist<1, 2>(ctx->stream, p, dy_hi, dy_lo, w_hi, w_lo, d->cin, cred / 8, dx_hi, dx_lo, skip_flags, out_flags, out_list, ctx->ws,
-                                  ctx->ws_bytes, !lazy_out);
+                                  ctx->ws_bytes, !lazy_out, ctx->sparse_chain_legacy != 0, next_flags, next_list, next_cols, &next_done);
     PP_CHECK_LAUNCH(ctx, "pp_conv2d_nhwc_bwd_data_bf16x3");
+    if (next_flags && !next_done)
+      return PP_API(pp_row_block_list_planes_within)(ctx, dx_hi, dx_lo, p.M, d->ld_x, next_cols, p.add_hi || p.addend ? nullptr : out_flags,
+                                                     next_flags, next_list);
     return PP_OK;
   }
   dispatch3(ctx, p, dy_hi, dy_lo, w_hi, w_lo, d->cin, cred / 8, dx_hi, dx_lo, chi, clo, skip_flags);
   PP_CHECK_LAUNCH(ctx, "pp_conv2d_nhwc_bwd_data_bf16x3");
+  if (next_flags) return PP_API(pp_row_block_list_planes_within)(ctx, dx_hi, dx_lo, p.M, d->ld_x, next_cols, nullptr, next_flags, next_list);
   return PP_OK;
 }
 namespace {
diff --git a/pyrapose_amd/csrc/ctx.hip b/pyrapose_amd/csrc/ctx.hip
--- a/pyrapose_amd/csrc/ctx.hip
+++ b/pyrapose_amd/csrc/ctx.hip
@@ -24,6 +24,8 @@
   c->n_cu = prop.multiProcessorCount;
   snprintf(c->name, sizeof(c->name), "%s (%s)", prop.name, prop.gcnArchName);
   c->err[0] = 0;
+  const char* chain = getenv("PP_SPARSE_CHAIN");
+  c->sparse_chain_legacy = (chain && strcmp(chain, "legacy") == 0) ? 1 : 0;
   *out = c;
   return PP_OK;
 }
@@ -78,6 +80,15 @@
   return PP_OK;
 }
 
+extern "C" int pp_ctx_set_row_block_flags_out(pp_ctx* ctx, unsigned char* flags, int* list, int cols) {
+  PP_REQUIRE_CTX(ctx);
+  PP_CHECK_ARG(ctx, (flags == nullptr) == (list == nullptr) && (!flags || cols > 0), PP_ERR_ARG, "pp_ctx_set_row_block_flags_out: flags, list and cols go together");
+  ctx->next_flags = flags;
+  ctx->next_list = list;
+  ctx->next_cols = cols;
+  return PP_OK;
+}
+
 extern "C" int pp_ctx_set_row_block_out(pp_ctx* ctx, const unsigned char* flags, int* list) {
   PP_REQUIRE_CTX(ctx);
   PP_CHECK_ARG(ctx, (flags == nullptr) == (list == nullptr), PP_ERR_ARG, "pp_ctx_set_row_block_out: flags and list go together");
diff --git a/pyrapose_amd/csrc/pp_internal.h b/pyrapose_amd/csrc/pp_internal.h
--- a/pyrapose_amd/csrc/pp_internal.h
+++ b/pyrapose_amd/csrc/pp_internal.h
@@ -25,6 +25,10 @@
   const unsigned char* out_flags;
   int* out_list;
   int planes_fmt;
+  unsigned char* next_flags;
+  int* next_list;
+  int next_cols;
+  int sparse_chain_legacy;
   const float* grad_scale;
 };
 
diff --git a/pyrapose_amd/engine.py b/pyrapose_amd/engine.py
--- a/pyrapose_amd/engine.py
+++ b/pyrapose_amd/engine.py
@@ -775,10 +775,17 @@
                     m_t, m_hi = (mask.t, None) if mask.t is not None else (None, mask.pl[0])
                 if gcap is not None:
                     assert dy_t is not None
+                hint = None
+                if lazy_out and _os.environ.get("PP_SPARSE_CHAIN", "") != "legacy":
+                    nb_ = (act.rows + 31) // 32
+                    producer["skip"] = (torch.zeros((2 * nb_,), dtype=torch.uint8, device="cuda"),
+                                        torch.zeros((2 * (nb_ + 1),), dtype=torch.int32, device="cuda"))
+                    producer["skip_made"] = True
+                    hint = (producer["skip"][0], producer["skip"][1], min((act.C + 3) // 4 * 4, act.ld))
                 self.bwd_ops.append(Op(lambda d=op["desc"], dy_t=dy_t, dy_pl=dy_pl, dh=pl["dg_hi"], dl=pl["dg_lo"], a_t=a_t, a_pl=a_pl, m_t=m_t,
-                                       m_hi=m_hi, out=out, gcap=gcap, sk=sk, lazy_out=lazy_out, lazy_in=lazy_in:
+                                       m_hi=m_hi, out=out, gcap=gcap, sk=sk, lazy_out=lazy_out, lazy_in=lazy_in, hint=hint:
                                        ops.conv_bwd_data3(ctx, d, dy_t, dh, dl, a_t, m_t, out.t, dy_pl, out.pl, gcap, sk, a_pl, m_hi,
-                                                          lazy_out=lazy_out, lazy_in=lazy_in), "conv_dgrad",
+                                                          lazy_out=lazy_out, lazy_in=lazy_in, hint_out=hint), "conv_dgrad",
                                        op["spec"].name, op["flops"]))
                 out.within = sk[0][sk[0].numel() // 2:] if (sk is not None and acc is None and _os.environ.get("PP_SPARSE_WITHIN", "1") != "0") else None
                 out.lazy = lazy_out
@@ -842,7 +849,9 @@
             if kind == "conv":
                 s, x = op["spec"], op["x"]
                 lctx = ctx.twin(y.fmt)
-                if self._sparse_layer(s) and g.contiguous() and len(g.shape()) == 2:
+                if op.get("skip_made"):
+                    assert self._sparse_layer(s) and g.lazy and g.pl is not None and g.shape() == (y.rows, y.ld), s.name
+                elif self._sparse_layer(s) and g.contiguous() and len(g.shape()) == 2:
                     nb = (g.shape()[0] + 31) // 32
                     skip = op["skip"] = (torch.zeros((2 * nb,), dtype=torch.uint8, device="cuda"),
                                          torch.zeros((2 * (nb + 1),), dtype=torch.int32, device="cuda"))
diff --git a/pyrapose_amd/ops.py b/pyrapose_amd/ops.py
--- a/pyrapose_amd/ops.py
+++ b/pyrapose_amd/ops.py
@@ -303,7 +303,10 @@
 
 
 def conv_bwd_data3(ctx, d, dy, w_hi, w_lo, addend, relu_src, dx, dy_planes=None, dx_planes=None, dy_capture=None, dy_skip=None,
-                   addend_planes=None, relu_src_hi=None, lazy_out=False, lazy_in=False):
+                   addend_planes=None, relu_src_hi=None, lazy_out=False, lazy_in=False, hint_out=None):
+    if hint_out is not None:
+        check(lib.pp_ctx_set_row_block_flags_out(ctx.handle, _ptr(hint_out[0]), _ptr(hint_out[1]), int(hint_out[2])), ctx.handle,
+              "pp_ctx_set_row_block_flags_out")
     _set_capture(ctx, dy_capture)
     _set_skip(ctx, dy_skip, lazy_out, lazy_in)
     _set_epilogue_planes(ctx, addend_planes, relu_src_hi)
```

Result: faster. 609.5, median of 6 (+1.0%).
